# geneo4PETSc/geneo4PETSc

Measured on AMD Instinct MI355X. Metric: GenEO-PCG setup+solve sec and SpMV GB/s, 3D Laplacian 50M DoF, 1/2/4/8 GPUs, higher is better.
Workload: dtype f64

## Files before the change

### geneo4petsc_amd/csrc/amg.cpp

```cpp
#include "amg.h"

#include <algorithm>
#include <atomic>
#include <chrono>
#include <memory>
#include <cmath>
#include <cstdio>
#include <cstdlib>
#include <functional>
#include <exception>
#include <mutex>
#include <stdexcept>
#include <thread>

#include "dense.h"

namespace geneo {

static std::atomic<int> g_null_pivots{0};
int amg_null_pivots_take() { return g_null_pivots.exchange(0); }

static void parallel_rows(int n, const std::function<void(int, int)>& f) {
  int nth = std::max(1, std::min(16, (int)std::thread::hardware_concurrency()));
  if (n < 20000) nth = 1;
  if (nth == 1) {
    f(0, n);
    return;
  }
  std::vector<std::thread> th;
  for (int t = 0; t < nth; ++t)
    th.emplace_back([&, t]() { f((int)((int64_t)n * t / nth), (int)((int64_t)n * (t + 1) / nth)); });
  for (auto& x : th) x.join();
}

static HostCsr transpose_blocks(const HostCsr& a, int ncols, const std::vector<int>& rs, const std::vector<int>& cs) {
  HostCsr t;
  t.n = ncols;
  t.rowptr.assign(ncols + 1, 0);
  for (int c : a.col) t.rowptr[c + 1]++;
  for (int i = 0; i < ncols; ++i) t.rowptr[i + 1] += t.rowptr[i];
  t.col.resize(a.col.size());
  t.val.resize(a.val.size());
  const int nb = (int)rs.size() - 1;
  auto one = [&](int b) {
    std::vector<int> fill(t.rowptr.begin() + cs[b], t.rowptr.begin() + cs[b + 1]);
    for (int i = rs[b]; i < rs[b + 1]; ++i)
      for (int k = a.rowptr[i]; k < a.rowptr[i + 1]; ++k) {
        const int p = fill[a.col[k] - cs[b]]++;
        t.col[p] = i;
        t.val[p] = a.val[k];
      }
  };
  std::vector<std::thread> th;
  for (int b = 0; b < nb; ++b) th.emplace_back(one, b);
  for (auto& x : th) x.join();
  return t;
}

static HostCsr transpose(const HostCsr& a, int ncols) {
  HostCsr t;
  t.n = ncols;
  t.rowptr.assign(ncols + 1, 0);
  for (int c : a.col) t.rowptr[c + 1]++;
  for (int i = 0; i < ncols; ++i) t.rowptr[i + 1] += t.rowptr[i];
  t.col.resize(a.col.size());
  t.val.resize(a.val.size());
  std::vector<int> fill(t.rowptr.begin(), t.rowptr.end() - 1);
  for (int i = 0; i < a.n; ++i)
    for (int k = a.rowptr[i]; k < a.rowptr[i + 1]; ++k) {
      const int p = fill[a.col[k]]++;
      t.col[p] = i;
      t.val[p] = a.val[k];
    }
  return t;
}

static HostCsr spgemm(const HostCsr& a, const HostCsr& b, int ncols_b) {
  const int n = a.n;
  HostCsr c;
  c.n = n;
  c.rowptr.assign(n + 1, 0);
  int nth = std::max(1, std::min(16, (int)std::thread::hardware_concurrency()));
  if (a.col.size() < 200000) nth = 1;
  nth = std::max(1, std::min(nth, n));
  std::vector<int> cut(nth + 1, n);
  cut[0] = 0;
  for (int t = 1; t < nth; ++t) {
    const int64_t target = (int64_t)a.rowptr[n] * t / nth;
    cut[t] = (int)(std::lower_bound(a.rowptr.begin(), a.rowptr.begin() + n + 1, (int)target) - a.rowptr.begin());
    cut[t] = std::min(n, std::max(cut[t], cut[t - 1]));
  }
  auto range = [&](int t, int& r0, int& r1) {
    r0 = cut[t];
    r1 = cut[t + 1];
  };
  auto run = [&](const std::function<void(int)>& f) {
    if (nth == 1) { f(0); return; }
// ... 434 lines not shown
    } else {
      if (l == 0) throw std::runtime_error("AMG: the level-0 matrix must already be resident (fine_dev)");
      L.A = bk::csr_upload(H.A.n, H.A.rowptr.data(), H.A.col.data(), H.A.val.data());
    }
    if (l + 1 < levels.size()) {
      L.P = bk::csr_upload(H.P.n, H.P.rowptr.data(), H.P.col.data(), H.P.val.data());
      bool ok = !getenv("GENEO_AMG_UPLOAD_R");
      if (ok) {
        L.R = bk::transpose(L.P, H.R.n, &ok);
        if (ok) bk::csr_finish(L.R);
      }
      if (!ok) L.R = bk::csr_upload(H.R.n, H.R.rowptr.data(), H.R.col.data(), H.R.val.data());
    }
    L.dinv = (double*)bk::alloc(sizeof(double) * std::max(1, L.n));
    bk::h2d(L.dinv, H.dinv.data(), sizeof(double) * L.n);
    alloc_level_buffers(L, l > 0);
    L.fused = bk::csr_fusable(L.A) && (l + 1 == (int)levels.size() || bk::csr_fusable(L.P)) && !getenv("GENEO_AMG_UNFUSED");
    if (l + 1 < levels.size()) {
      make_column_scaled(L);
      make_post_matrix(L, nullptr, levels[l + 1].n);
    }
    if (l == 0) nnz0 = (double)H.nnz;
    nnzt += (double)H.nnz;
    L.suboff = H.suboff;
    lv.push_back(L);
  }
  opc = nnz0 > 0 ? nnzt / nnz0 : 1.0;
  const AmgLevelHost& C = levels.back();
  cch = bk::chunks_upload((int)C.suboff.size() - 1, C.suboff.data());
  d_inv = (double*)bk::alloc(sizeof(double) * std::max<size_t>(1, coarse_inv.size()));
  bk::h2d(d_inv, coarse_inv.data(), sizeof(double) * coarse_inv.size());
  d_invbase = (int64_t*)bk::alloc(sizeof(int64_t) * coarse_base.size());
  bk::h2d(d_invbase, coarse_base.data(), sizeof(int64_t) * coarse_base.size());
  if (prm.single) make_single();
}

void AmgDevice::make_single() {
  nlp = 0;
  for (Lvl& L : lv) {
    if (!L.fused) continue;
    const bool had = bk::csr_has_lp(L.A);
    if (bk::csr_make_lp(L.A)) ++nlp;
    L.own_lp_A = !L.own_A && !had && bk::csr_has_lp(L.A);
    if (L.Acs.n && bk::csr_make_lp(L.Acs, &L.A)) ++nlp;
    if (L.P.n && bk::csr_make_lp(L.P)) ++nlp;
    if (L.R.n && bk::csr_make_lp(L.R)) ++nlp;
    if (L.M.n && bk::csr_make_lp(L.M)) ++nlp;
  }
}

double AmgDevice::jacobi_weight(const Lvl& L) const {
  const double lmax = 1.1 * L.rho, lmin = lmax / std::max(1.5, prm.smooth_ratio);
  return 1.0 / (0.5 * (lmax + lmin));
}

void AmgDevice::make_post_matrix(Lvl& L, bk::Csr* ap, int nc) {
  const bool want = prm.smooth_degree <= 1 && L.fused && !getenv("GENEO_AMG_NO_POST_MATRIX");
  bk::Csr AP;
  bool ok = true;
  if (ap) AP = *ap;
  else if (want) AP = bk::spgemm(L.A, L.P, nc, &ok);
  if (!want || !ok || AP.n == 0) {
    if (AP.n) bk::csr_free(AP);
    return;
  }
  if (!bk::post_matrix(AP, L.P, L.dinv, jacobi_weight(L))) {
    bk::csr_free(AP);
    return;
  }
  bk::csr_finish(AP);
  if (!bk::csr_fusable(AP)) {
    bk::csr_free(AP);
    return;
  }
  L.M = AP;
}

void AmgDevice::make_column_scaled(Lvl& L) {
  if (L.fused && L.A.vec_lpr == 0 && L.A.nlong == 0 && L.A.n > 0 && !getenv("GENEO_AMG_NO_PRESCALE"))
    L.Acs = bk::csr_scaled_alias(L.A, nullptr, L.dinv, true);
}

void AmgDevice::alloc_level_buffers(Lvl& L, bool coarse) {
  const size_t blk = sizeof(double) * std::max<size_t>(1, (size_t)L.n * maxm);
  L.r = (double*)bk::alloc(blk);
  L.d = (double*)bk::alloc(blk);
  if (prm.smooth_degree > 1) L.ad = (double*)bk::alloc(blk);
  if (coarse) {
    L.b = (double*)bk::alloc(blk);
    L.x = (double*)bk::alloc(blk);
  }
}

AmgLevelHostPart amg_level_host_part(const HostCsr& Ah, const std::vector<int>& so, const AmgParams& prm, int l) {
  AmgLevelHostPart h;
  const int nsub = (int)so.size() - 1;
  const auto t_hp0 = std::chrono::high_resolution_clock::now();
  h.rho = gershgorin_rho(Ah, h.dinv, so);
  const auto t_hp1 = std::chrono::high_resolution_clock::now();
  int maxblk = 0;
  for (int s = 0; s < nsub; ++s) maxblk = std::max(maxblk, so[s + 1] - so[s]);
  h.last = (maxblk <= prm.coarse_size || l + 1 >= prm.max_levels);
  h.csub.assign(nsub + 1, 0);
  if (!h.last) {
    const int n = Ah.n;
    h.agg.assign(n, -1);
    std::vector<int> nagg(nsub, 0);
    std::vector<std::thread> th;
    for (int s = 0; s < nsub; ++s)
      th.emplace_back([&, s]() { nagg[s] = aggregate_block(Ah, so[s], so[s + 1], h.agg, amg_strength(prm, l), aggregate_threads(nsub)); });
    for (auto& x : th) x.join();
    for (int s = 0; s < nsub; ++s) h.csub[s + 1] = h.csub[s] + nagg[s];
    for (int s = 1; s < nsub; ++s) {
      const int off = h.csub[s];
      parallel_rows(so[s + 1] - so[s], [&](int a0, int a1) {
        for (int i = so[s] + a0; i < so[s] + a1; ++i) h.agg[i] += off;
      });
    }
    h.nc = h.csub[nsub];
    if (h.nc >= n) h.last = true;
  }
  if (getenv("GENEO_DEBUG") && Ah.n > 500000)
    fprintf(stderr, "[amg/host] level %d, %d rows: diagonal + bound %.3f s, aggregation %.3f s\n", l, Ah.n,
            std::chrono::duration<double>(t_hp1 - t_hp0).count(),
            std::chrono::duration<double>(std::chrono::high_resolution_clock::now() - t_hp1).count());
  return h;
}

namespace {
struct HostCsrPool {
  std::mutex mu;
  std::vector<HostCsr> parked;
  static constexpr size_t MAX_PARKED = 12;
  HostCsr take(int n, size_t nnz) {
    HostCsr out;
    {
      std::lock_guard<std::mutex> lk(mu);
      int best = -1;
      for (size_t i = 0; i < parked.size(); ++i) {
        const HostCsr& h = parked[i];
        if (h.col.size() == nnz && h.rowptr.size() == (size_t)n + 1) { best = (int)i; break; }
        if (h.col.capacity() >= nnz && h.rowptr.capacity() >= (size_t)n + 1 &&
            (best < 0 || h.col.capacity() < parked[best].col.capacity()))
          best = (int)i;
      }
      if (best >= 0) {
        out = std::move(parked[best]);
        parked.erase(parked.begin() + best);
      }
    }
    out.n = n;
    out.rowptr.resize((size_t)n + 1);
    out.col.resize(nnz);
    out.val.resize(nnz);
    return out;
  }
  void give(HostCsr&& h) {
    if (h.col.capacity() < (1u << 16)) return;
    std::lock_guard<std::mutex> lk(mu);
    if (parked.size() >= MAX_PARKED) {
      size_t k = 0;
      for (size_t i = 1; i < parked.size(); ++i)
        if (parked[i].col.capacity() < parked[k].col.capacity()) k = i;
      if (parked[k].col.capacity() >= h.col.capacity()) return;
      parked.erase(parked.begin() + k);
    }
    parked.push_back(std::move(h));
  }
};
HostCsrPool g_host_csr_pool;
}

bool AmgDevice::build_on_device(const HostCsr& A, const std::vector<int>& suboff, const AmgParams& p, int max_m,
// ... 213 lines not shown
```

### geneo4petsc_amd/csrc/backend_hip.hip

```cpp
#include <hip/hip_runtime.h>

#include <algorithm>
#include <atomic>
#include <cstdio>
#include <cstdlib>
#include <functional>
#include <stdexcept>
#include <string>
#include <chrono>
#include <condition_variable>
#include <cstring>
#include <thread>
#include <type_traits>
#include <map>
#include <mutex>
#include <unordered_map>
#include <vector>

#include "backend.h"
#include "cheb_dev.h"

#define HIPCHK(x)                                                                          \
  do {                                                                                     \
    hipError_t e_ = (x);                                                                   \
    if (e_ != hipSuccess) {                                                                \
      throw std::runtime_error(std::string("HIP error ") + hipGetErrorString(e_) + " at " + \
                               __FILE__ + ":" + std::to_string(__LINE__));                 \
    }                                                                                      \
  } while (0)

namespace bk {

static hipStream_t g_stream_main = nullptr;
static thread_local hipStream_t t_stream_side = nullptr;
static thread_local bool t_side = false;
static thread_local bool g_capturing = false;
static thread_local hipStream_t g_capture_stream = nullptr;
static std::atomic<int> g_device{-1};
static thread_local bool t_dev_bound = false;
static inline void bind_thread() {
  if (t_dev_bound) return;
  t_dev_bound = true;
  const int want = g_device.load(std::memory_order_acquire);
  if (want < 0) {
    int d = 0;
    if (hipGetDevice(&d) == hipSuccess) g_device.store(d, std::memory_order_release);
    else (void)hipGetLastError();
  } else {
    int d = -1;
    if (hipGetDevice(&d) != hipSuccess || d != want) {
      if (hipSetDevice(want) != hipSuccess) throw std::runtime_error("geneo: hipSetDevice failed on a library thread");
    }
  }
}
static inline hipStream_t stream_cur() {
  bind_thread();
  return g_capturing ? g_capture_stream : (t_side ? t_stream_side : g_stream_main);
}
#define g_stream (stream_cur())
static bool g_no_mfma = false;
static bool g_spgemm_fill_scan = getenv("GENEO_SPGEMM_SCAN_FILL") != nullptr;
static bool g_gram_flat = getenv("GENEO_GRAM_NO_FLAT") == nullptr;
static bool g_init = false;
__device__ int g_lp_no_fixed = 0;
static bool g_sell_offsets = !(getenv("GENEO_SELL_OFFSETS") && atoi(getenv("GENEO_SELL_OFFSETS")) == 0);

static void lazy_init() {
  if (g_init) return;
  g_init = true;
  const char* e = getenv("GENEO_NO_MFMA");
  g_no_mfma = (e && e[0] == '1');
  if (const char* f = getenv("GENEO_LP_FIXED")) {
    const int off = atoi(f) ? 0 : 1;
    (void)hipMemcpyToSymbol(HIP_SYMBOL(g_lp_no_fixed), &off, sizeof(int));
  }
}

const char* name() { return "hip-gfx950"; }
void set_stream(void* s) {
  if ((hipStream_t)s != g_stream_main) (void)hipStreamSynchronize(g_stream_main);
  g_stream_main = (hipStream_t)s;
  int d = 0;
  if (hipGetDevice(&d) == hipSuccess) g_device.store(d, std::memory_order_release);
  else (void)hipGetLastError();
  t_dev_bound = true;
}
void side_stream_begin(void* after, bool use_after) {
  if (t_side) return;
  bind_thread();
  if (!t_stream_side) HIPCHK(hipStreamCreateWithFlags(&t_stream_side, hipStreamNonBlocking));
  hipEvent_t ev;
  HIPCHK(hipEventCreateWithFlags(&ev, hipEventDisableTiming));
  HIPCHK(hipEventRecord(ev, use_after ? (hipStream_t)after : g_stream_main));
  HIPCHK(hipStreamWaitEvent(t_stream_side, ev, 0));
  (void)hipEventDestroy(ev);
  t_side = true;
}
void side_stream_end() {
  if (!t_side) return;
  (void)hipStreamSynchronize(t_stream_side);
  t_side = false;
  (void)hipStreamDestroy(t_stream_side);
  t_stream_side = nullptr;
}
void* get_stream() { return (void*)g_stream; }
void sync() { HIPCHK(hipStreamSynchronize(g_stream)); }

int device_count() {
  int n = 0;
  if (hipGetDeviceCount(&n) != hipSuccess) { (void)hipGetLastError(); return 0; }
  return n;
}
int set_device(int ordinal) {
  const int n = device_count();
  if (n <= 0 || ordinal < 0) return -1;
  const int d = ordinal % n;
  if (hipSetDevice(d) != hipSuccess) { (void)hipGetLastError(); return -1; }
  g_device.store(d, std::memory_order_release);
  t_dev_bound = true;
  return d;
}
int current_device() { return g_device.load(std::memory_order_acquire); }
int thread_device_check() {
  int got = -2;
  std::thread t([&]() {
    try {
      (void)stream_cur();
      int d = -1;
      if (hipGetDevice(&d) == hipSuccess) got = d;
    } catch (...) {
      got = -3;
    }
  });
  t.join();
  return got;
}
static double g_alloc_s = 0.0, g_free_s = 0.0;
static long long g_alloc_n = 0;
static std::mutex g_alloc_mu;
static std::unordered_map<void*, size_t> g_live;
struct Parked { void* p; hipStream_t stream; hipEvent_t ev; };
static std::multimap<size_t, Parked> g_cache;
static std::vector<hipEvent_t> g_ev_pool;
static size_t g_cache_bytes = 0;
static size_t g_live_bytes = 0, g_live_peak = 0, g_foot_peak = 0;
static inline void mem_account(long long delta_live) {
  g_live_bytes = (size_t)((long long)g_live_bytes + delta_live);
  g_live_peak = std::max(g_live_peak, g_live_bytes);
  g_foot_peak = std::max(g_foot_peak, g_live_bytes + g_cache_bytes);
}
static bool alloc_cache_on() {
  static const bool on = !(getenv("GENEO_ALLOC_CACHE") && !strcmp(getenv("GENEO_ALLOC_CACHE"), "0"));
  return on;
}
static size_t alloc_cache_cap() {
  static const size_t cap = (size_t)((getenv("GENEO_ALLOC_CACHE_GB") ? atof(getenv("GENEO_ALLOC_CACHE_GB")) : 96.0) * 1073741824.0);
  return cap;
}
static inline size_t alloc_round(size_t bytes) {
  const size_t g = bytes < ((size_t)1 << 20) ? 512 : ((size_t)2 << 20);
  return (bytes + g - 1) / g * g;
}
void alloc_cache_release() {
  bind_thread();
  std::lock_guard<std::mutex> lk(g_alloc_mu);
  if (g_cache.empty()) return;
  auto t0 = std::chrono::high_resolution_clock::now();
  (void)hipDeviceSynchronize();
  for (auto& kv : g_cache) {
    (void)hipFree(kv.second.p);
    if (kv.second.ev) g_ev_pool.push_back(kv.second.ev);
  }
  g_cache.clear();
  g_cache_bytes = 0;
  g_free_s += std::chrono::duration<double>(std::chrono::high_resolution_clock::now() - t0).count();
}
void* alloc(size_t bytes) {
  lazy_init();
  bind_thread();
  void* p = nullptr;
  if (bytes == 0) bytes = 8;
  const size_t sz = alloc_cache_on() ? alloc_round(bytes) : bytes;
  if (alloc_cache_on()) {
    std::lock_guard<std::mutex> lk(g_alloc_mu);
    auto it = g_cache.lower_bound(sz);
    if (it != g_cache.end() && it->first <= sz + sz / 8 + 4096) {
      p = it->second.p;
      if (it->second.ev) {
        if (it->second.stream != g_stream) (void)hipStreamWaitEvent(g_stream, it->second.ev, 0);
        g_ev_pool.push_back(it->second.ev);
      }
      g_live[p] = it->first;
      g_cache_bytes -= it->first;
      mem_account((long long)it->first);
      g_cache.erase(it);
    }
  }
  if (!p) {
    auto t0 = std::chrono::high_resolution_clock::now();
    hipError_t e = hipMalloc(&p, sz);
    if (e != hipSuccess && alloc_cache_on()) {
      (void)hipGetLastError();
      alloc_cache_release();
      e = hipMalloc(&p, sz);
    }
    HIPCHK(e);
    const double dt = std::chrono::duration<double>(std::chrono::high_resolution_clock::now() - t0).count();
    static const bool trace = getenv("GENEO_ALLOC_TRACE") != nullptr;
    if (trace && dt > 2e-4) fprintf(stderr, "[alloc] %.1f MB in %.3f ms\n", sz / 1e6, dt * 1e3);
    std::lock_guard<std::mutex> lk(g_alloc_mu);
    g_alloc_s += dt;
    ++g_alloc_n;
    g_live[p] = sz;
    mem_account((long long)sz);
  }
  HIPCHK(hipMemsetAsync(p, 0, bytes, g_stream));
  return p;
}
void dfree(void* p) {
  if (!p) return;
  bind_thread();
  {
    std::lock_guard<std::mutex> lk(g_alloc_mu);
    auto it = g_live.find(p);
    if (it != g_live.end()) {
      const size_t sz = it->second;
      g_live.erase(it);
      mem_account(-(long long)sz);
      if (alloc_cache_on() && g_cache_bytes + sz <= alloc_cache_cap()) {
        Parked pk{p, g_stream, nullptr};
        if (!g_capturing) {
          if (!g_ev_pool.empty()) { pk.ev = g_ev_pool.back(); g_ev_pool.pop_back(); }
          else if (hipEventCreateWithFlags(&pk.ev, hipEventDisableTiming) != hipSuccess) pk.ev = nullptr;
          if (pk.ev && hipEventRecord(pk.ev, g_stream) != hipSuccess) { g_ev_pool.push_back(pk.ev); pk.ev = nullptr; }
        }
        g_cache.emplace(sz, pk);
        g_cache_bytes += sz;
        return;
      }
    }
  }
  auto t0 = std::chrono::high_resolution_clock::now();
  (void)hipFree(p);
  g_free_s += std::chrono::duration<double>(std::chrono::high_resolution_clock::now() - t0).count();
}
void mem_info(double* live, double* live_peak, double* footprint_peak, double* cached, double* dev_free, double* dev_total,
              bool reset_peaks) {
  bind_thread();
  size_t f = 0, t = 0;
  if (hipMemGetInfo(&f, &t) != hipSuccess) { (void)hipGetLastError(); f = t = 0; }
  std::lock_guard<std::mutex> lk(g_alloc_mu);
  if (live) *live = (double)g_live_bytes;
  if (live_peak) *live_peak = (double)g_live_peak;
  if (footprint_peak) *footprint_peak = (double)g_foot_peak;
  if (cached) *cached = (double)g_cache_bytes;
  if (dev_free) *dev_free = (double)f;
  if (dev_total) *dev_total = (double)t;
  if (reset_peaks) {
    g_live_peak = g_live_bytes;
    g_foot_peak = g_live_bytes + g_cache_bytes;
  }
}
void alloc_stats(double* alloc_s, double* free_s, long long* n) {
  *alloc_s = g_alloc_s; *free_s = g_free_s; *n = g_alloc_n;
  g_alloc_s = g_free_s = 0.0; g_alloc_n = 0;
}
constexpr size_t STAGE_BYTES = (size_t)16 << 20;
struct StageSet {
  char* buf[2] = {nullptr, nullptr};
  hipEvent_t ev[2];
  bool ready = false, busy = false, failed = false;
};
static StageSet g_stage_sets[2];
static std::mutex g_stage_mu;
static std::condition_variable g_stage_cv;
static StageSet* stage_acquire() {
  if (getenv("GENEO_NO_PINNED_STAGING")) return nullptr;
  bind_thread();
  std::unique_lock<std::mutex> lk(g_stage_mu);
  for (;;) {
    bool any_usable = false;
    for (StageSet& st : g_stage_sets) {
      if (st.failed) continue;
      any_usable = true;
      if (st.busy) continue;
      if (!st.ready) {
        bool ok = true;
        for (int i = 0; i < 2 && ok; ++i) {
          if (hipHostMalloc((void**)&st.buf[i], STAGE_BYTES, hipHostMallocDefault) != hipSuccess) {
            (void)hipGetLastError();
            if (i == 1) (void)hipHostFree(st.buf[0]);
            st.buf[0] = st.buf[1] = nullptr;
            ok = false;
          } else if (hipEventCreateWithFlags(&st.ev[i], hipEventDisableTiming) != hipSuccess) {
            ok = false;
          }
        }
        if (!ok) { st.failed = true; continue; }
        st.ready = true;
      }
      st.busy = true;
// ... 129 lines not shown
}
void graph_destroy(void* exec) {
  if (!exec) return;
  graph_counts_drop(exec);
  (void)hipGraphExecDestroy((hipGraphExec_t)exec);
}

static inline int cdiv(int64_t a, int64_t b) { return (int)((a + b - 1) / b); }
static inline int grid1d(int64_t n, int per_block) {
  int g = cdiv(n, per_block);
  return g < 1 ? 1 : g;
}

static inline int gridv(int64_t n) { return std::min(grid1d(n, 1024), 2048); }

__device__ __forceinline__ double wave_sum(double v) {
#pragma unroll
  for (int o = 32; o > 0; o >>= 1) v += __shfl_down(v, o, 64);
  return v;
}
__device__ __forceinline__ double block_sum_256(double v, double* sm ) {
  v = wave_sum(v);
  const int w = threadIdx.x >> 6, l = threadIdx.x & 63;
  __syncthreads();
  if (l == 0) sm[w] = v;
  __syncthreads();
  return sm[0] + sm[1] + sm[2] + sm[3];
}
constexpr int SPMV_TILE = 1792;
constexpr int SPMV_ROWS = 256;
constexpr int SELL_LONG = 64;
constexpr int SELL_VEC_MAX_ROWS = 1 << 18;

__global__ void k_slice_width(const int* __restrict__ rowptr, int n, int ns, int* __restrict__ w, int long_len) {
  const int s = blockIdx.x * blockDim.x + threadIdx.x;
  if (s >= ns) return;
  int m = 0;
  const int r1 = (64 * s + 64 < n) ? 64 * s + 64 : n;
  for (int i = 64 * s; i < r1; ++i) {
    const int len = rowptr[i + 1] - rowptr[i];
    if (len <= long_len && len > m) m = len;
  }
  w[s] = m;
}
__global__ __launch_bounds__(256) void k_sell_fill(const int* __restrict__ rowptr, const int* __restrict__ col,
                                                   const double* __restrict__ val, int n, int ns,
                                                   const int64_t* __restrict__ sl_ptr, int* __restrict__ sl_col,
                                                   double* __restrict__ sl_val, int long_len) {
  const int s = blockIdx.x * 4 + (threadIdx.x >> 6);
  if (s >= ns) return;
  const int l = threadIdx.x & 63;
  const int i = 64 * s + l;
  const int64_t base = sl_ptr[s];
  const int w = (int)((sl_ptr[s + 1] - base) >> 6);
  int a = 0, len = 0;
  if (i < n) {
    a = rowptr[i];
    len = rowptr[i + 1] - a;
  }
  const bool use = (i < n) && len <= long_len;
  int padc = 0;
  if (i < n && len > 0) padc = use ? col[a + len - 1] : col[a];
  else if (n > 0 && rowptr[n] > 0) {
    const int k = (i < n) ? a : rowptr[n];
    padc = col[k > 0 ? k - 1 : 0];
  }
  for (int k = 0; k < w; ++k) {
    const int64_t e = base + (int64_t)64 * k + l;
    if (use && k < len) {
      sl_col[e] = col[a + k];
      sl_val[e] = val[a + k];
    } else {
      sl_col[e] = padc;
      sl_val[e] = 0.0;
    }
  }
}

int spmv_kind();
static bool g_force_slices = false;
static void finish_layout(Csr& a, const int* h_rowptr, const int* h_col = nullptr);

Csr csr_upload_raw(int n, const int* h_rowptr, const int* h_col, const double* h_val) {
  Csr a;
  a.n = n;
  a.nnz = h_rowptr[n];
  a.rowptr = (int*)alloc(sizeof(int) * (size_t)(n + 1));
  a.col = (int*)alloc(sizeof(int) * std::max<size_t>(1, (size_t)a.nnz));
  a.val = (double*)alloc(sizeof(double) * std::max<size_t>(1, (size_t)a.nnz));
  h2d(a.rowptr, h_rowptr, sizeof(int) * (size_t)(n + 1));
  h2d(a.col, h_col, sizeof(int) * (size_t)a.nnz);
  h2d(a.val, h_val, sizeof(double) * (size_t)a.nnz);
  return a;
}
__global__ void k_iota_ones(int* __restrict__ rp, double* __restrict__ val, int n) {
  for (int i = blockIdx.x * blockDim.x + threadIdx.x; i <= n; i += gridDim.x * blockDim.x) {
    rp[i] = i;
    if (i < n) val[i] = 1.0;
  }
}
Csr csr_tentative_prolongator(int n, const int* agg_dev) {
  Csr a;
  a.n = n;
  a.nnz = n;
  a.rowptr = (int*)alloc(sizeof(int) * (size_t)(n + 1));
  a.col = (int*)alloc(sizeof(int) * std::max<size_t>(1, (size_t)n));
  a.val = (double*)alloc(sizeof(double) * std::max<size_t>(1, (size_t)n));
  hipLaunchKernelGGL(k_iota_ones, dim3(grid1d(n + 1, 256)), dim3(256), 0, stream_cur(), a.rowptr, a.val, n);
  if (n > 0) d2d(a.col, agg_dev, sizeof(int) * (size_t)n);
  return a;
}
Csr csr_upload(int n, const int* h_rowptr, const int* h_col, const double* h_val) {
  Csr a;
  a.n = n;
  a.nnz = h_rowptr[n];
  a.rowptr = (int*)alloc(sizeof(int) * (size_t)(n + 1));
  a.col = (int*)alloc(sizeof(int) * std::max<size_t>(1, (size_t)a.nnz));
  a.val = (double*)alloc(sizeof(double) * std::max<size_t>(1, (size_t)a.nnz));
  static const bool dbg = getenv("GENEO_DEBUG") != nullptr;
  auto t0 = std::chrono::high_resolution_clock::now();
  h2d(a.rowptr, h_rowptr, sizeof(int) * (size_t)(n + 1));
  h2d(a.col, h_col, sizeof(int) * (size_t)a.nnz);
  h2d(a.val, h_val, sizeof(double) * (size_t)a.nnz);
  auto t1 = std::chrono::high_resolution_clock::now();
  finish_layout(a, h_rowptr, h_col);
  if (dbg && a.nnz > 4000000) {
    HIPCHK(hipStreamSynchronize(g_stream));
    auto t2 = std::chrono::high_resolution_clock::now();
    fprintf(stderr, "[upload] n %d nnz %lld: copies %.4f s (%.1f GB/s), layouts %.4f s\n", n, (long long)a.nnz,
            std::chrono::duration<double>(t1 - t0).count(),
            (12.0 * a.nnz + 4.0 * n) / std::chrono::duration<double>(t1 - t0).count() / 1e9,
            std::chrono::duration<double>(t2 - t1).count());
  }
  return a;
}
static std::vector<int> strip_schedule(int nslice, const std::vector<int>& frow) {
  const int WT = std::max(64, getenv("GENEO_SPMM_STRIP") ? atoi(getenv("GENEO_SPMM_STRIP")) : 3072);
  std::vector<int> order;
  order.reserve(nslice);
  int64_t covered = 0;
  std::vector<std::vector<int>> bucket;
  for (int sa = 0; sa < nslice;) {
    int sb = sa + 1;
    while (sb < nslice && frow[sb] == frow[sa]) ++sb;
    const int F = frow[sa];
    const bool swept = F >= 4 * WT && (int64_t)(sb - sa) * 64 >= (int64_t)3 * F;
    if (!swept) {
      for (int s = sa; s < sb; ++s) order.push_back(s);
    } else {
      const int nst = std::max(1, (F + WT / 2) / WT);
      const int W = (F + nst - 1) / nst;
      bucket.assign(nst, {});
      for (int s = sa; s < sb; ++s) bucket[(int)((((int64_t)(s - sa) * 64) % F) / W)].push_back(s);
      for (int b = 0; b < nst; ++b) order.insert(order.end(), bucket[b].begin(), bucket[b].end());
      covered += sb - sa;
    }
    sa = sb;
  }
  if (covered * 10 < (int64_t)nslice * 8) return {};
  if (getenv("GENEO_DEBUG_SCHED"))
    fprintf(stderr, "[sched] strip: %d slices, %lld swept, far offset of the first run %d rows, strip target %d rows\n", nslice,
            (long long)covered, frow[0], WT);
  return order;
}

static std::vector<int> blob_schedule(int n, const int* h_rowptr, const int* h_col, int nslice) {
  const int TILE = std::max(4, getenv("GENEO_SPMM_TILE") ? atoi(getenv("GENEO_SPMM_TILE")) : 512);
  const char* mode = getenv("GENEO_SPMM_SCHED");
  if (mode && !strcmp(mode, "natural")) return {};
  if (nslice < 4 * TILE) return {};
  std::vector<int> adj_ptr((size_t)nslice + 1, 0), adj;
  constexpr int CAP = 60;
  const int nth = std::max(1, std::min(8, nslice / 4096));
  std::vector<std::vector<int>> part_adj(nth);
  std::vector<int> part_far(nth, 0);
  std::vector<int> cnts((size_t)nslice, 0);
  std::vector<int> frow((size_t)nslice, 0);
  auto sample = [&](int t) {
    const int s0 = (int)((int64_t)nslice * t / nth), s1 = (int)((int64_t)nslice * (t + 1) / nth);
    std::vector<int>& out = part_adj[t];
    out.reserve((size_t)(s1 - s0) * 8);
    int far_t = 0;
    for (int s = s0; s < s1; ++s) {
      int loc[64];
      int cnt = 0;
      const int r0 = 64 * s, r1 = std::min(n, r0 + 64);
      const int probe[4] = {r0, r0 + 21, r0 + 42, r1 - 1};
      for (int t4 = 0; t4 < 4; ++t4) {
        const int r = std::min(probe[t4], r1 - 1);
        for (int k = h_rowptr[r]; k < h_rowptr[r + 1] && cnt < CAP; ++k) {
          frow[s] = std::max(frow[s], std::abs(h_col[k] - r));
          const int o = h_col[k] >> 6;
          if (o == s || o >= nslice) continue;
          bool seen = false;
          for (int i = 0; i < cnt; ++i) seen = seen || loc[i] == o;
          if (!seen) loc[cnt++] = o;
        }
      }
      for (int i = 0; i < cnt; ++i) {
        out.push_back(loc[i]);
        far_t = std::max(far_t, std::abs(loc[i] - s));
      }
      cnts[s] = cnt;
    }
    part_far[t] = far_t;
  };
  if (nth > 1) {
    std::vector<std::thread> th;
    for (int t = 1; t < nth; ++t) th.emplace_back(sample, t);
    sample(0);
    for (auto& x : th) x.join();
  } else {
    sample(0);
  }
  int far = 0;
  for (int t = 0; t < nth; ++t) far = std::max(far, part_far[t]);
  for (int s = 0; s < nslice; ++s) adj_ptr[s + 1] = adj_ptr[s] + cnts[s];
  if (!(mode && !strcmp(mode, "blob")) && far < TILE / 4) return {};
  if (!(mode && !strcmp(mode, "blob"))) {
    std::vector<int> order = strip_schedule(nslice, frow);
    if (!order.empty()) return order;
  }
  adj.reserve((size_t)adj_ptr[nslice]);
  for (int t = 0; t < nth; ++t) adj.insert(adj.end(), part_adj[t].begin(), part_adj[t].end());
  std::vector<int> order;
  order.reserve(nslice);
  std::vector<char> seen((size_t)nslice, 0);
  std::vector<int> queue;
  int next_seed = 0;
  while ((int)order.size() < nslice) {
    while (next_seed < nslice && seen[next_seed]) ++next_seed;
    if (next_seed >= nslice) break;
    queue.clear();
    queue.push_back(next_seed);
    seen[next_seed] = 1;
    size_t head = 0;
    int taken = 0;
    while (head < queue.size() && taken < TILE) {
      const int s = queue[head++];
      order.push_back(s);
      ++taken;
      for (int k = adj_ptr[s]; k < adj_ptr[s + 1]; ++k) {
        const int o = adj[k];
        if (!seen[o]) { seen[o] = 1; queue.push_back(o); }
      }
    }
    for (; head < queue.size(); ++head) seen[queue[head]] = 0;
  }
  return order;
}

static void finish_layout(Csr& a, const int* h_rowptr, const int* h_col) {
  const int n = a.n;
  static const bool dbg_l = getenv("GENEO_DEBUG") != nullptr;
  auto tl0 = std::chrono::high_resolution_clock::now();
  auto lapl = [&](const char* what) {
    if (!dbg_l || a.nnz < 4000000) return;
    HIPCHK(hipStreamSynchronize(g_stream));
    auto t = std::chrono::high_resolution_clock::now();
    fprintf(stderr, "[layout] %-22s %.4f s\n", what, std::chrono::duration<double>(t - tl0).count());
    tl0 = t;
  };
  int maxrow = 0;
  std::vector<int> longr;
  const int long_len = SELL_LONG;
  for (int i = 0; i < n; ++i) {
    const int len = h_rowptr[i + 1] - h_rowptr[i];
    maxrow = std::max(maxrow, len);
    if (len > long_len) longr.push_back(i);
  }
  a.max_row = maxrow;
  lapl("row lengths (host)");
  if (spmv_kind() == 0) {
    std::vector<int> blk;
    blk.push_back(0);
    int r = 0;
    while (r < n) {
      int r1 = r;
      int nz = 0;
      while (r1 < n && (r1 - r) < SPMV_ROWS) {
        const int len = h_rowptr[r1 + 1] - h_rowptr[r1];
        if (nz + len > SPMV_TILE) break;
        nz += len;
        ++r1;
      }
      if (r1 == r) ++r1;
      blk.push_back(r1);
      r = r1;
    }
    a.nblk = (int)blk.size() - 1;
    a.rowblk = (int*)alloc(sizeof(int) * blk.size());
    h2d(a.rowblk, blk.data(), sizeof(int) * blk.size());
  }
  {
    const int ns = (n + 63) / 64;
    int* dw = (int*)alloc(sizeof(int) * std::max(1, ns));
    if (ns > 0)
      hipLaunchKernelGGL(k_slice_width, dim3(grid1d(ns, 256)), dim3(256), 0, g_stream, a.rowptr, n, ns, dw, long_len);
    std::vector<int> w(std::max(1, ns));
    d2h(w.data(), dw, sizeof(int) * ns);
    dfree(dw);
    std::vector<int64_t> sp(ns + 1, 0);
    for (int s = 0; s < ns; ++s) sp[s + 1] = sp[s] + (int64_t)64 * w[s];
    a.nslice = ns;
    a.sl_nnz = sp[ns];
    a.sl_ptr = (int64_t*)alloc(sizeof(int64_t) * (ns + 1));
    a.sl_col = (int*)alloc(sizeof(int) * (size_t)std::max<int64_t>(1, sp[ns]));
    a.sl_val = (double*)alloc(sizeof(double) * (size_t)std::max<int64_t>(1, sp[ns]));
    h2d(a.sl_ptr, sp.data(), sizeof(int64_t) * (ns + 1));
    lapl("slice widths + scan");
    if (ns > 0)
      hipLaunchKernelGGL(k_sell_fill, dim3((ns + 3) / 4), dim3(256), 0, g_stream, a.rowptr, a.col, a.val, n, ns,
                         a.sl_ptr, a.sl_col, a.sl_val, long_len);
    lapl("slice fill");
    {
      int xp[9];
      for (int g = 0; g <= 8; ++g) xp[g] = (int)(((int64_t)ns * g) / 8);
      a.xcd_ptr = (int*)alloc(sizeof(int) * 9);
      h2d(a.xcd_ptr, xp, sizeof(int) * 9);
      if (h_col && longr.empty()) {
        const std::vector<int> order = blob_schedule(n, h_rowptr, h_col, ns);
        if ((int)order.size() == ns) {
          a.sched = (int*)alloc(sizeof(int) * (size_t)ns);
          h2d(a.sched, order.data(), sizeof(int) * (size_t)ns);
        }
      }
    }
    lapl("blob schedule");
    a.nlong = (int)longr.size();
    const double avg = n > 0 ? (double)a.nnz / n : 0.0;
    static const int vec_max_rows = getenv("GENEO_SELL_VEC_MAX_ROWS") ? atoi(getenv("GENEO_SELL_VEC_MAX_ROWS")) : SELL_VEC_MAX_ROWS;
    if (!g_force_slices && n < vec_max_rows && (a.nlong > 0 || avg >= 20.0)) a.vec_lpr = avg <= 24.0 ? 16 : (avg <= 48.0 ? 32 : 64);
    a.long_rows = (int*)alloc(sizeof(int) * std::max<size_t>(1, longr.size()));
    h2d(a.long_rows, longr.data(), sizeof(int) * longr.size());
  }
// ... 307 lines not shown
    const unsigned long long prev = __shfl_up(ck, 1, 64);
    const bool head = (ck != ~0ull) && (lane == 0 || (prev >> 6) != (ck >> 6));
    double acc = 0.0 + v;
    for (int d = 1; d < 64; ++d) {
      const unsigned long long nk = __shfl_down(ck, d, 64);
      const double nv = __shfl_down(v, d, 64);
      const bool more = head && lane + d < 64 && (nk >> 6) == (ck >> 6);
      if (more) acc += nv;
      if (!__ballot(more)) break;
    }
    const unsigned long long heads = __ballot(head);
    if (head) {
      const int pos = __builtin_popcountll(heads & ((1ull << lane) - 1ull));
      ccol[base + pos] = (int)(ck >> 6);
      cval[base + pos] = acc;
    }
    return;
  }
  spg_collect(arp, acol, brp, bcol, row, lane, keys[w], ja[w], pre[w], total, overflow);
  const int* kw = keys[w];
  double* hv = hval[w];
  for (int s = lane; s < SPG_HS; s += 64) hv[s] = 0.0;
  if (lane == 0) cntl[w] = 0;
  for (int t = lane; t < SPG_MAXD; t += 64) list[w][t] = 0x7fffffff;
  __builtin_amdgcn_fence(__ATOMIC_ACQ_REL, "wavefront");
  __builtin_amdgcn_wave_barrier();
  const int a0 = arp[row], na = arp[row + 1] - a0;
  if (total >= 0) {
    constexpr int NB = 4;
    for (int p0 = 0; p0 < total; p0 += 64 * NB) {
      int kk[NB], slot[NB];
      double vv[NB];
#pragma unroll
      for (int t = 0; t < NB; ++t) {
        const int p = p0 + 64 * t + lane;
        kk[t] = (p < total) ? spg_find(pre[w], na, p) : 0x7fffffff;
      }
#pragma unroll
      for (int t = 0; t < NB; ++t) {
        slot[t] = 0;
        vv[t] = 0.0;
        if (kk[t] != 0x7fffffff) {
          const int l = brp[ja[w][kk[t]]] + (p0 + 64 * t + lane - pre[w][kk[t]]);
          slot[t] = bcol[l];
          vv[t] = aval[a0 + kk[t]] * bval[l];
        }
      }
#pragma unroll
      for (int t = 0; t < NB; ++t)
        if (kk[t] != 0x7fffffff) slot[t] = spg_lookup(kw, slot[t]);
#pragma unroll
      for (int t = 0; t < NB; ++t) {
        if (p0 + 64 * t >= total) break;
        int kc = __builtin_amdgcn_readfirstlane(kk[t]);
        while (true) {
          if (kk[t] == kc) hv[slot[t]] += vv[t];
          __builtin_amdgcn_fence(__ATOMIC_ACQ_REL, "wavefront");
          const unsigned long long later = __ballot(kk[t] != 0x7fffffff && kk[t] > kc);
          if (!later) break;
          kc = __shfl(kk[t], __builtin_ctzll(later), 64);
        }
      }
    }
  } else {
    for (int k = a0; k < a0 + na; ++k) {
      const int j = acol[k];
      const double av = aval[k];
      for (int l = brp[j] + lane; l < brp[j + 1]; l += 64) hv[spg_lookup(kw, bcol[l])] += av * bval[l];
      __builtin_amdgcn_fence(__ATOMIC_ACQ_REL, "wavefront");
    }
  }
  __builtin_amdgcn_fence(__ATOMIC_ACQ_REL, "wavefront");
  __builtin_amdgcn_wave_barrier();
  for (int s = lane; s < SPG_HS; s += 64) {
    const int key = kw[s];
    if (key != -1) {
      const int t = atomicAdd(&cntl[w], 1);
      list[w][t] = key;
      lval[w][t] = hv[s];
    }
  }
  __builtin_amdgcn_fence(__ATOMIC_ACQ_REL, "wavefront");
  __builtin_amdgcn_wave_barrier();
  int N = 64;
  while (N < cnt) N <<= 1;
  wave_bitonic_sort(list[w], lval[w], N, lane);
  for (int t = lane; t < cnt; t += 64) {
    ccol[base + t] = list[w][t];
    cval[base + t] = lval[w][t];
  }
}
template <int G, bool FILL>
__global__ __launch_bounds__(256) void k_spgemm_small(int n, const int* __restrict__ arp, const int* __restrict__ acol,
                                                      const double* __restrict__ aval, const int* __restrict__ brp,
                                                      const int* __restrict__ bcol, const double* __restrict__ bval,
                                                      int* __restrict__ cnt, const int* __restrict__ crp,
                                                      int* __restrict__ ccol, double* __restrict__ cval,
                                                      unsigned char* __restrict__ defer, int* __restrict__ flags) {
  constexpr int RPW = 64 / G;
  const int w = threadIdx.x >> 6, lane = threadIdx.x & 63;
  const int gl = lane % G, gbase = lane - gl;
  const int row = (blockIdx.x * 4 + w) * RPW + lane / G;
  const bool live = row < n;
  const int a0 = live ? arp[row] : 0;
  const int na = live ? arp[row + 1] - a0 : 0;
  int b0 = 0, len = 0;
  double av = 0.0;
  if (gl < na && na <= G) {
    const int j = acol[a0 + gl];
    b0 = brp[j];
    len = brp[j + 1] - b0;
    if (FILL) av = aval[a0 + gl];
  }
  int incl = len;
#pragma unroll
  for (int o = 1; o < G; o <<= 1) {
    const int t = __shfl_up(incl, o, G);
    if (gl >= o) incl += t;
  }
  const int total = __shfl(incl, G - 1, G);
  const bool fits = na <= G && total <= G;
  if (!FILL && live && gl == 0) {
    defer[row] = fits ? 0 : 1;
    if (!fits) atomicAdd(&flags[1], 1);
  }
  int k = 0;
#pragma unroll
  for (int q = 0; q < G; ++q) k += (__shfl(incl, q, G) <= gl) ? 1 : 0;
  const bool has = fits && gl < total;
  const int ks = has ? k : 0;
  const int kb0 = __shfl(b0, ks, G);
  const int kexcl = __shfl(incl - len, ks, G);
  double kav = 0.0;
  if (FILL) kav = __shfl(av, ks, G);
  unsigned long long ck = ~0ull;
  double v = 0.0;
  if (has) {
    const int l = kb0 + (gl - kexcl);
    ck = ((unsigned long long)(unsigned)bcol[l] << 6) | (unsigned)gl;
    if (FILL) v = kav * bval[l];
  }
#pragma unroll
  for (int k2 = 2; k2 <= G; k2 <<= 1)
#pragma unroll
    for (int j = k2 >> 1; j > 0; j >>= 1) {
      const unsigned long long ock = __shfl_xor(ck, j, 64);
      double ov = 0.0;
      if (FILL) ov = __shfl_xor(v, j, 64);
      const bool take_min = (((gl & j) == 0) == ((gl & k2) == 0));
      const bool swap = take_min ? (ock < ck) : (ock > ck);
      if (swap) { ck = ock; if (FILL) v = ov; }
    }
  const unsigned long long prev = __shfl_up(ck, 1, G);
  const bool head = (ck != ~0ull) && (gl == 0 || (prev >> 6) != (ck >> 6));
  const unsigned long long gmask = (G == 64) ? ~0ull : (((1ull << G) - 1ull) << gbase);
  const unsigned long long heads = __ballot(head) & gmask;
  if (!FILL) {
    if (live && fits && gl == 0) cnt[row] = __builtin_popcountll(heads);
    return;
  }
  double acc = 0.0 + v;
  for (int d = 1; d < G; ++d) {
    const unsigned long long nk = __shfl_down(ck, d, G);
    const double nv = __shfl_down(v, d, G);
    const bool more = head && gl + d < G && (nk >> 6) == (ck >> 6);
    if (more) acc += nv;
// ... 36 lines not shown
  }
  if (t == 255) totals[blockIdx.x] = part[255];
}
__global__ __launch_bounds__(256) void k_scan_blocks64(int64_t* __restrict__ x, int64_t n, int64_t* __restrict__ totals) {
  __shared__ int64_t part[256];
  const int64_t b0 = (int64_t)blockIdx.x * SCAN_B;
  const int t = threadIdx.x;
  int64_t v[4], run = 0;
#pragma unroll
  for (int u = 0; u < 4; ++u) {
    const int64_t i = b0 + 4 * t + u;
    run += (i < n) ? x[i] : 0;
    v[u] = run;
  }
  part[t] = run;
  __syncthreads();
  for (int o = 1; o < 256; o <<= 1) {
    const int64_t add = (t >= o) ? part[t - o] : 0;
    __syncthreads();
    part[t] += add;
    __syncthreads();
  }
  const int64_t before = (t > 0) ? part[t - 1] : 0;
#pragma unroll
  for (int u = 0; u < 4; ++u) {
    const int64_t i = b0 + 4 * t + u;
    if (i < n) x[i] = before + v[u];
  }
  if (t == 255) totals[blockIdx.x] = part[255];
}
__global__ void k_scan_add(int* __restrict__ x, int64_t n, const int64_t* __restrict__ totals_incl) {
  for (int64_t i = (int64_t)blockIdx.x * blockDim.x + threadIdx.x + SCAN_B; i < n; i += (int64_t)gridDim.x * blockDim.x)
    x[i] += (int)totals_incl[i / SCAN_B - 1];
}
__global__ void k_scan_add64(int64_t* __restrict__ x, int64_t n, const int64_t* __restrict__ totals_incl) {
  for (int64_t i = (int64_t)blockIdx.x * blockDim.x + threadIdx.x + SCAN_B; i < n; i += (int64_t)gridDim.x * blockDim.x)
    x[i] += totals_incl[i / SCAN_B - 1];
}
static void device_inclusive_scan64(int64_t* x, int64_t n) {
  if (n <= 0) return;
  const int64_t nb = (n + SCAN_B - 1) / SCAN_B;
  int64_t* tot = (int64_t*)alloc(sizeof(int64_t) * (size_t)nb);
  hipLaunchKernelGGL(k_scan_blocks64, dim3((unsigned)nb), dim3(256), 0, g_stream, x, n, tot);
  if (nb > 1) {
    t_sp_report.scan_depth = 2;
    device_inclusive_scan64(tot, nb);
    hipLaunchKernelGGL(k_scan_add64, dim3((unsigned)std::min<int64_t>(nb, 4096)), dim3(256), 0, g_stream, x, n, tot);
  }
  dfree(tot);
}
static void host_exclusive_scan(int* dcnt_to_ptr, int n, int64_t* total) {
  if (n <= 0) { *total = 0; return; }
  static const bool on_host = getenv("GENEO_SCAN_HOST") != nullptr;
  if (on_host || (int64_t)n < 4 * SCAN_B) {
    std::vector<int> h((size_t)n + 1, 0);
    d2h(h.data() + 1, dcnt_to_ptr + 1, sizeof(int) * (size_t)n);
    int64_t run = 0;
    for (int i = 1; i <= n; ++i) {
      run += h[i];
      h[i] = (int)run;
    }
    h[0] = 0;
    h2d(dcnt_to_ptr, h.data(), sizeof(int) * ((size_t)n + 1));
    *total = run;
    return;
  }
  int* x = dcnt_to_ptr + 1;
  t_sp_report.scan_depth = 1;
  const int64_t nb = ((int64_t)n + SCAN_B - 1) / SCAN_B;
  int64_t* tot = (int64_t*)alloc(sizeof(int64_t) * (size_t)nb);
  hipLaunchKernelGGL(k_scan_blocks, dim3((unsigned)nb), dim3(256), 0, g_stream, x, (int64_t)n, tot);
  device_inclusive_scan64(tot, nb);
  hipLaunchKernelGGL(k_scan_add, dim3((unsigned)std::min<int64_t>(nb, 4096)), dim3(256), 0, g_stream, x, (int64_t)n, tot);
  HIPCHK(hipMemsetAsync(dcnt_to_ptr, 0, sizeof(int), g_stream));
  int64_t run = 0;
  d2h(&run, tot + (nb - 1), sizeof(int64_t));
  dfree(tot);
  if (run > 0x7fffffffLL) throw std::runtime_error("sparse product: more than 2^31 entries");
  *total = run;
}
static bool g_spgemm_small_host = true;
Csr spgemm(const Csr& a, const Csr& b, int ncols_b, bool* ok) {
  (void)ncols_b;
  Csr c;
  *ok = true;
  t_sp_report = SparseProductReport();
  c.n = a.n;
  if (a.n == 0) return c;
  int* dflag = (int*)alloc(2 * sizeof(int));
  c.rowptr = (int*)alloc(sizeof(int) * ((size_t)a.n + 1));
  int G = 0;
  if (g_spgemm_small_host && !g_spgemm_fill_scan && a.n >= 256 && b.n > 0) {
    const double na = (double)a.nnz / a.n, est = na * ((double)b.nnz / b.n);
    if (na <= 7.5 && est <= 7.5) G = 8;
    else if (na <= 15.0 && est <= 14.0) G = 16;
    else if (na <= 30.0 && est <= 26.0) G = 32;
    else if (na <= 60.0 && est <= 52.0) G = 64;
  }
  t_sp_report.group = G;
  unsigned char* defer = nullptr;
#define SPG_SMALL(GG, FILL)                                                                                                  \
  hipLaunchKernelGGL((k_spgemm_small<GG, FILL>), dim3((unsigned)((a.n + 256 / GG - 1) / (256 / GG))), dim3(256), 0, g_stream, \
                     a.n, a.rowptr, a.col, a.val, b.rowptr, b.col, b.val, c.rowptr + 1, c.rowptr, c.col, c.val, defer, dflag)
#define SPG_SMALL_G(FILL)                                      \
  do {                                                         \
    if (G == 8) SPG_SMALL(8, FILL);                            \
    else if (G == 16) SPG_SMALL(16, FILL);                     \
    else if (G == 32) SPG_SMALL(32, FILL);                     \
    else SPG_SMALL(64, FILL);                                  \
  } while (0)
  int hflag[2] = {0, 0};
  if (G) {
    defer = (unsigned char*)alloc((size_t)a.n);
    SPG_SMALL_G(false);
    d2h(hflag, dflag, 2 * sizeof(int));
    t_sp_report.deferred = hflag[1];
  }
  const bool general = !G || hflag[1] > 0;
  if (general) {
    hipLaunchKernelGGL(k_spgemm_count, dim3((a.n + 3) / 4), dim3(256), 0, g_stream, a.n, a.rowptr, a.col, b.rowptr, b.col,
                       c.rowptr + 1, dflag, defer);
    d2h(hflag, dflag, sizeof(int));
  }
  if (hflag[0]) {
    dfree(dflag);
    dfree(defer);
    dfree(c.rowptr);
    *ok = false;
    return Csr();
  }
  int64_t total = 0;
  host_exclusive_scan(c.rowptr, a.n, &total);
  c.nnz = total;
  c.col = (int*)alloc(sizeof(int) * std::max<size_t>(1, (size_t)total));
  c.val = (double*)alloc(sizeof(double) * std::max<size_t>(1, (size_t)total));
  if (G) SPG_SMALL_G(true);
  if (general) {
    if (g_spgemm_fill_scan)
      hipLaunchKernelGGL(k_spgemm_fill_scan, dim3((a.n + 3) / 4), dim3(256), 0, g_stream, a.n, a.rowptr, a.col, a.val, b.rowptr,
                         b.col, b.val, c.rowptr, c.col, c.val, dflag);
    else
      hipLaunchKernelGGL(k_spgemm_fill, dim3((a.n + 3) / 4), dim3(256), 0, g_stream, a.n, a.rowptr, a.col, a.val, b.rowptr,
                         b.col, b.val, c.rowptr, c.col, c.val, dflag, defer);
    d2h(hflag, dflag, sizeof(int));
  }
#undef SPG_SMALL_G
#undef SPG_SMALL
  dfree(dflag);
  dfree(defer);
  if (hflag[0]) {
    dfree(c.rowptr); dfree(c.col); dfree(c.val);
    *ok = false;
    return Csr();
  }
  return c;
}

constexpr int TR_MAXROW = 1024;
__global__ void k_col_count(const int* __restrict__ col, int64_t nnz, int* __restrict__ cnt) {
  for (int64_t e = (int64_t)blockIdx.x * blockDim.x + threadIdx.x; e < nnz; e += (int64_t)gridDim.x * blockDim.x)
    atomicAdd(&cnt[col[e]], 1);
}
__global__ void k_tr_scatter(int n, const int* __restrict__ rp, const int* __restrict__ col, const double* __restrict__ val,
                             const int* __restrict__ trp, int* __restrict__ cursor, int* __restrict__ tcol,
                             double* __restrict__ tval) {
  for (int i = blockIdx.x * blockDim.x + threadIdx.x; i < n; i += gridDim.x * blockDim.x)
    for (int k = rp[i]; k < rp[i + 1]; ++k) {
      const int c = col[k];
      const int p = trp[c] + atomicAdd(&cursor[c], 1);
      tcol[p] = i;
      tval[p] = val[k];
    }
}
__global__ __launch_bounds__(256) void k_sort_rows(int n, const int* __restrict__ rp, int* __restrict__ col,
                                                   double* __restrict__ val, int* __restrict__ overflow) {
  __shared__ int key[4][TR_MAXROW];
  __shared__ double v[4][TR_MAXROW];
  const int w = threadIdx.x >> 6, lane = threadIdx.x & 63;
  const int row = blockIdx.x * 4 + w;
  if (row >= n) return;
  const int base = rp[row], cnt = rp[row + 1] - base;
  if (cnt <= 1) return;
  if (cnt > TR_MAXROW) {
    if (lane == 0) *overflow = 1;
    return;
  }
  int N = 64;
  while (N < cnt) N <<= 1;
  for (int t = lane; t < N; t += 64) {
    key[w][t] = (t < cnt) ? col[base + t] : 0x7fffffff;
    v[w][t] = (t < cnt) ? val[base + t] : 0.0;
  }
  __builtin_amdgcn_wave_barrier();
  wave_bitonic_sort(key[w], v[w], N, lane);
  for (int t = lane; t < cnt; t += 64) {
    col[base + t] = key[w][t];
    val[base + t] = v[w][t];
  }
}
Csr transpose(const Csr& a, int ncols, bool* ok) {
  Csr t;
  *ok = true;
  t_sp_report = SparseProductReport();
  t.n = ncols;
  t.nnz = a.nnz;
  t.rowptr = (int*)alloc(sizeof(int) * ((size_t)ncols + 1));
  t.col = (int*)alloc(sizeof(int) * std::max<size_t>(1, (size_t)a.nnz));
  t.val = (double*)alloc(sizeof(double) * std::max<size_t>(1, (size_t)a.nnz));
  if (a.nnz > 0)
    hipLaunchKernelGGL(k_col_count, dim3(gridv(a.nnz)), dim3(256), 0, g_stream, a.col, (int64_t)a.nnz, t.rowptr + 1);
  int64_t total = 0;
  host_exclusive_scan(t.rowptr, ncols, &total);
  int* cursor = (int*)alloc(sizeof(int) * std::max<size_t>(1, (size_t)ncols));
  int* dflag = (int*)alloc(sizeof(int));
  if (a.n > 0)
    hipLaunchKernelGGL(k_tr_scatter, dim3(gridv(a.n)), dim3(256), 0, g_stream, a.n, a.rowptr, a.col, a.val, t.rowptr,
                       cursor, t.col, t.val);
  if (ncols > 0)
    hipLaunchKernelGGL(k_sort_rows, dim3((ncols + 3) / 4), dim3(256), 0, g_stream, ncols, t.rowptr, t.col, t.val, dflag);
  int hflag = 0;
  d2h(&hflag, dflag, sizeof(int));
  dfree(dflag);
  dfree(cursor);
  if (hflag) {
    dfree(t.rowptr); dfree(t.col); dfree(t.val);
    *ok = false;
    return Csr();
  }
  return t;
}
__global__ void k_smooth_p(int n, const int* __restrict__ rp, const int* __restrict__ col, double* __restrict__ val,
                           const int* __restrict__ agg, const double* __restrict__ dinv, double w) {
  for (int i = blockIdx.x * blockDim.x + threadIdx.x; i < n; i += gridDim.x * blockDim.x) {
    const double f = -w * dinv[i];
    const int mine = agg[i];
    for (int k = rp[i]; k < rp[i + 1]; ++k) val[k] = f * val[k] + (col[k] == mine ? 1.0 : 0.0);
  }
}
void smooth_prolongator(Csr& ap0, const int* agg_dev, const double* dinv_dev, double w) {
  if (ap0.n == 0) return;
  hipLaunchKernelGGL(k_smooth_p, dim3(gridv(ap0.n)), dim3(256), 0, g_stream, ap0.n, ap0.rowptr, ap0.col, ap0.val, agg_dev,
                     dinv_dev, w);
}

__global__ void k_post_matrix(int n, const int* __restrict__ arp, const int* __restrict__ acol, double* __restrict__ aval,
                              const int* __restrict__ prp, const int* __restrict__ pcol, const double* __restrict__ pval,
                              const double* __restrict__ dinv, double w, int* __restrict__ miss) {
  for (int i = blockIdx.x * blockDim.x + threadIdx.x; i < n; i += gridDim.x * blockDim.x) {
    const int p0 = prp[i], p1 = prp[i + 1];
    const double f = w * dinv[i];
    int found = 0;
    for (int k = arp[i]; k < arp[i + 1]; ++k) {
      const int c = acol[k];
      double v = -f * aval[k];
      for (int q = p0; q < p1; ++q)
        if (pcol[q] == c) { v += pval[q]; ++found; break; }
      aval[k] = v;
    }
    if (found != p1 - p0) atomicExch(miss, 1);
  }
}
bool post_matrix(Csr& ap, const Csr& p, const double* dinv, double w) {
  if (ap.n == 0) return true;
  int* dmiss = (int*)alloc(sizeof(int));
  hipLaunchKernelGGL(k_post_matrix, dim3(gridv(ap.n)), dim3(256), 0, g_stream, ap.n, ap.rowptr, ap.col, ap.val, p.rowptr,
                     p.col, p.val, dinv, w, dmiss);
  int miss = 0;
  d2h(&miss, dmiss, sizeof(int));
  dfree(dmiss);
  return miss == 0;
}

void csr_free_lp(Csr& a) {
  dfree(a.lp_val);
  if (!a.alias) { dfree(a.lp_col); dfree(a.lp_base); dfree(a.off_mask); dfree(a.off_rec); }
  a.lp_val = nullptr; a.lp_col = nullptr; a.lp_base = nullptr;
  a.off_mask = nullptr; a.off_rec = nullptr; a.off_coded = 0; a.off_nnz = 0;
}
void csr_free(Csr& a) {
  csr_free_lp(a);
  if (a.alias) {
    dfree(a.val); dfree(a.sl_val);
    a = Csr();
    return;
  }
  dfree(a.rowptr); dfree(a.col); dfree(a.val); dfree(a.rowblk);
  dfree(a.sl_ptr); dfree(a.sl_col); dfree(a.sl_val); dfree(a.long_rows);
  dfree(a.sched); dfree(a.xcd_ptr);
  a = Csr();
}

__global__ void k_scale_csr(int n, const int* __restrict__ rowptr, const int* __restrict__ col, const double* __restrict__ val,
                            const double* __restrict__ rs, const double* __restrict__ cs, double* __restrict__ out) {
  const int r = blockIdx.x * blockDim.x + threadIdx.x;
  if (r >= n) return;
  const double a = rs ? rs[r] : 1.0;
  for (int k = rowptr[r]; k < rowptr[r + 1]; ++k) out[k] = a * val[k] * (cs ? cs[col[k]] : 1.0);
}
__global__ __launch_bounds__(256) void k_scale_sell(int n, int ns, const int64_t* __restrict__ sl_ptr,
                                                    const int* __restrict__ sl_col, const double* __restrict__ sl_val,
                                                    const double* __restrict__ rs, const double* __restrict__ cs,
                                                    double* __restrict__ out) {
  const int s = blockIdx.x * 4 + (threadIdx.x >> 6);
  if (s >= ns) return;
  const int l = threadIdx.x & 63;
  const int r = 64 * s + l;
  const double a = (rs && r < n) ? rs[r] : 1.0;
  for (int64_t e = sl_ptr[s] + l; e < sl_ptr[s + 1]; e += 64) out[e] = a * sl_val[e] * (cs ? cs[sl_col[e]] : 1.0);
}
Csr csr_scaled_alias(const Csr& a, const double* row_scale, const double* col_scale, bool col_is_dinv) {
  Csr b = a;
  b.alias = true;
  b.lp_val = nullptr; b.lp_col = nullptr; b.lp_base = nullptr;
  b.off_mask = nullptr; b.off_rec = nullptr; b.off_coded = 0; b.off_nnz = 0;
  b.col_scaled = col_is_dinv;
  b.val = (double*)alloc(sizeof(double) * std::max<size_t>(1, (size_t)a.nnz));
  b.sl_val = (double*)alloc(sizeof(double) * (size_t)std::max<int64_t>(1, a.sl_nnz));
  if (a.n > 0)
    hipLaunchKernelGGL(k_scale_csr, dim3(grid1d(a.n, 256)), dim3(256), 0, g_stream, a.n, a.rowptr, a.col, a.val, row_scale,
                       col_scale, b.val);
  if (a.nslice > 0)
    hipLaunchKernelGGL(k_scale_sell, dim3((a.nslice + 3) / 4), dim3(256), 0, g_stream, a.n, a.nslice, a.sl_ptr, a.sl_col,
                       a.sl_val, row_scale, col_scale, b.sl_val);
  return b;
}

__device__ __forceinline__ int xcd_remap(int b, int nblk) {
  const int per = (nblk + 7) >> 3;
  const int t = (b & 7) * per + (b >> 3);
  return t;
}

__global__ __launch_bounds__(256) void k_spmv_lds(const int* __restrict__ rowblk, int nblk,
                                                  const int* __restrict__ rowptr,
                                                  const int* __restrict__ col,
                                                  const double* __restrict__ val,
                                                  const double* __restrict__ x, double* __restrict__ y) {
  __shared__ double prod[SPMV_TILE];
  const int t = xcd_remap(blockIdx.x, nblk);
  if (t >= nblk) return;
  const int r0 = rowblk[t], r1 = rowblk[t + 1];
  const int nz0 = rowptr[r0], nz1 = rowptr[r1];
  const int cnt = nz1 - nz0;
  const int tid = threadIdx.x;
  if (cnt > SPMV_TILE) {
    double s = 0.0;
    for (int k = nz0 + tid; k < nz1; k += 256) s += val[k] * x[col[k]];
    prod[tid] = s;
    __syncthreads();
    for (int w = 128; w > 0; w >>= 1) {
      if (tid < w) prod[tid] += prod[tid + w];
      __syncthreads();
    }
    if (tid == 0) y[r0] = prod[0];
    return;
  }
  for (int k = tid; k < cnt; k += 256) prod[k] = val[nz0 + k] * x[col[nz0 + k]];
  __syncthreads();
  const int r = r0 + tid;
  if (r < r1) {
    const int a = rowptr[r] - nz0, b = rowptr[r + 1] - nz0;
    double s = 0.0;
    for (int k = a; k < b; ++k) s += prod[k];
    y[r] = s;
  }
}

__device__ __forceinline__ int4 lp_base_of(const int* __restrict__ base, int s) {
  return base ? reinterpret_cast<const int4*>(base)[s] : int4{0, 0, 0x7fffffff, 0};
}
template <typename COLT, bool NT>
struct ColsStored {
  const COLT* __restrict__ col;
  int4 cb;
  __device__ __forceinline__ int at(int u, int64_t e0) const {
    return (u < cb.z ? cb.x : cb.y) + (int)(NT ? __builtin_nontemporal_load(col + e0 + 64 * u) : col[e0 + 64 * u]);
  }
  template <int KW>
  __device__ __forceinline__ void finish(int (&)[KW]) const {}
};
constexpr int OFF_NONE = (int)0x80000000;
struct ColsOffset {
  int4 o0, o1;
  unsigned char m8;
  int ov;
  int r, pad;
  __device__ __forceinline__ int at(int, int64_t) const { return 0; }
  template <int KW>
  __device__ __forceinline__ void finish(int (&c)[KW]) const {
    constexpr unsigned full = (1u << KW) - 1u;
    const unsigned m = m8;
    const int off[8] = {o0.x, o0.y, o0.z, o0.w, o1.x, o1.y, o1.z, o1.w};
    if (__ballot(m != full) == 0) {
#pragma unroll
      for (int u = 0; u < KW; ++u) c[u] = r + off[u];
    } else {
      unsigned mm = m;
#pragma unroll
      for (int u = 0; u < KW; ++u) {
// ... 452 lines not shown
  const int s = blockIdx.x * 4 + (threadIdx.x >> 6);
  if (s >= ns) return;
  const int l = threadIdx.x & 63;
  const int r = 64 * s + l;
  const int64_t a = sl_ptr[s];
  const int wd = (int)((sl_ptr[s + 1] - a) >> 6);
  int len = r < n ? rowptr[r + 1] - rowptr[r] : 0;
  bool ok = wd >= 1 && wd <= 8 && __ballot(len > wd) == 0;
  if (!ok) len = 0;
  int d[8];
  int hi = -1;
#pragma unroll
  for (int k = 0; k < 8; ++k) {
    d[k] = 0;
    if (k < len) {
      const int c = sl_col[a + 64 * (int64_t)k + l];
      d[k] = c - r;
      hi = c > hi ? c : hi;
    }
  }
  hi = lp_wave_max(hi);
  int offs[8];
  int nd = 0, last = OFF_NONE;
#pragma unroll
  for (int it = 0; it < 9; ++it) {
    int mine = 0x7fffffff;
#pragma unroll
    for (int k = 0; k < 8; ++k)
      if (k < len && d[k] > last && d[k] < mine) mine = d[k];
    const int m = lp_wave_min(mine);
    const bool found = m != 0x7fffffff;
    if (it < 8) {
      offs[it < 8 ? it : 0] = found ? m : 0;
      if (found) nd = it + 1;
    } else if (found) {
      ok = false;
    }
    if (found) last = m;
  }
  unsigned msk = 0;
  int prev = -1;
  bool bad = false;
#pragma unroll
  for (int k = 0; k < 8; ++k) {
    if (k < len) {
      int slot = -1;
#pragma unroll
      for (int j = 0; j < 8; ++j)
        if (j < nd && offs[j] == d[k]) slot = j;
      if (slot <= prev) bad = true;
      else msk |= 1u << slot;
      prev = slot;
    }
  }
  const int pad = r < n ? r : n - 1;
  unsigned mm = bad ? 0u : msk;
#pragma unroll
  for (int k = 0; k < 8; ++k) {
    if (k < wd && ok) {
      int c = pad;
      if (mm) {
        const int slot = __ffs(mm) - 1;
        int o = 0;
#pragma unroll
        for (int j = 0; j < 8; ++j)
          if (j == slot) o = offs[j];
        c = r + o;
        mm &= mm - 1u;
      }
      if (k < len ? c != sl_col[a + 64 * (int64_t)k + l] : (c < 0 || c > hi)) bad = true;
    }
  }
  ok = ok && __ballot(bad) == 0;
  mask[r] = ok ? (unsigned char)msk : (unsigned char)0;
#pragma unroll
  for (int j = 0; j < 8; ++j)
    if (l == j) rec[8 * (int64_t)s + j] = ok ? offs[j] : OFF_NONE;
  if (ok && l == 0) {
    atomicAdd(cnt, 1ull);
    atomicAdd(cnt + 1, (unsigned long long)wd * 64ull);
  }
}
bool csr_make_lp(Csr& a, const Csr* index_owner) {
  if (spmv_kind() != 1 || a.nslice == 0 || !a.sl_ptr || a.vec_lpr > 0 || a.nlong > 0 || a.lp_val) return a.lp_val != nullptr;
  if (index_owner) {
    if (!index_owner->lp_val || index_owner->sl_col != a.sl_col) return false;
    a.lp_col = index_owner->lp_col;
    a.lp_base = index_owner->lp_base;
    a.off_mask = index_owner->off_mask;
    a.off_rec = index_owner->off_rec;
    a.off_coded = index_owner->off_coded;
    a.off_nnz = index_owner->off_nnz;
  } else {
    const char* lim_env = getenv("GENEO_LP_SPAN_MAX");
    int limit = lim_env ? atoi(lim_env) : 65535;
    if (limit < 1 || limit > 65535) limit = 65535;
    a.lp_base = (int*)alloc(sizeof(int4) * (size_t)a.nslice);
    unsigned long long* dstat = (unsigned long long*)alloc(3 * sizeof(unsigned long long));
    HIPCHK(hipMemsetAsync(dstat, 0, 3 * sizeof(unsigned long long), g_stream));
    int* dfail = (int*)dstat;
    unsigned long long* dcnt = dstat + 1;
    hipLaunchKernelGGL(k_lp_base, dim3((a.nslice + 3) / 4), dim3(256), 0, g_stream, a.nslice, a.sl_ptr, a.sl_col,
                       (int4*)a.lp_base, dfail, limit, dfail + 1);
    const double avg_w = (double)a.sl_nnz / (64.0 * (double)a.nslice);
    const bool off_try = a.rowptr && (a.max_row <= 8 || avg_w - 8.0 <= 0.1 * ((double)a.max_row - 8.0));
    if (off_try) {
      a.off_mask = (unsigned char*)alloc((size_t)64 * (size_t)a.nslice);
      a.off_rec = (int*)alloc(sizeof(int) * 8 * (size_t)a.nslice);
      hipLaunchKernelGGL(k_off_code, dim3((a.nslice + 3) / 4), dim3(256), 0, g_stream, a.nslice, a.n, a.rowptr, a.sl_ptr,
                         a.sl_col, a.off_mask, a.off_rec, dcnt);
    }
    unsigned long long hstat[3] = {0, 0, 0};
    d2h(hstat, dstat, sizeof(hstat));
    dfree(dstat);
    int hfail[2];
    memcpy(hfail, &hstat[0], sizeof(hfail));
    const unsigned long long* hcnt = hstat + 1;
    if (hfail[0]) {
      dfree(a.lp_base);
      a.lp_base = nullptr;
    } else {
      a.lp_col = (unsigned short*)alloc(sizeof(unsigned short) * (size_t)std::max<int64_t>(1, a.sl_nnz));
      a.off_coded = (int)hcnt[0];
      a.off_nnz = (int64_t)hcnt[1];
    }
    const bool off_use = a.lp_col && a.off_coded > 0 && 10 * (int64_t)a.off_coded >= 9 * (int64_t)a.nslice;
    if (!off_use) {
      dfree(a.off_mask);
      dfree(a.off_rec);
      a.off_mask = nullptr;
      a.off_rec = nullptr;
    }
    if (getenv("GENEO_DEBUG"))
      fprintf(stderr, "[offsets] %d-row matrix, %d slices, %d coded%s\n", a.n, a.nslice, a.off_coded,
              !off_try ? " (too wide: not tried)" : off_use ? "" : (a.off_coded ? " (under 90 %: stored columns kept)" : ""));
    if (getenv("GENEO_DEBUG") && (hfail[0] || hfail[1]))
      fprintf(stderr, "[lp] %d-row matrix, %d slices: %s (span limit %d)\n", a.n, a.nslice,
              hfail[0] ? "32-bit columns kept (a slice needs more than two bases)"
                       : (std::to_string(hfail[1]) + " slices with two column bases").c_str(), limit);
  }
  a.lp_val = (float*)alloc(sizeof(float) * (size_t)std::max<int64_t>(1, a.sl_nnz));
  hipLaunchKernelGGL(k_lp_fill, dim3((a.nslice + 3) / 4), dim3(256), 0, g_stream, a.nslice, a.sl_ptr, a.sl_col, a.sl_val,
                     (const int4*)a.lp_base, (index_owner || !a.lp_col) ? (unsigned short*)nullptr : a.lp_col, a.lp_val);
  return true;
}
template <int EPI, int WPS, typename COLT, bool NT, bool OFFS = false>
__global__ __launch_bounds__(256) void k_spmv_sell_lp(const int64_t* __restrict__ sl_ptr, int nslice, int n,
                                                      const COLT* __restrict__ col, const float* __restrict__ val,
                                                      const int* __restrict__ base, const double* __restrict__ x,
                                                      double* __restrict__ y, const double* __restrict__ b,
                                                      double* __restrict__ z, const double* __restrict__ dinv, double w,
                                                      const double* __restrict__ cs,
                                                      const unsigned char* __restrict__ omask = nullptr,
                                                      const int* __restrict__ orec = nullptr) {
  spmv_sell_slice<float, COLT, EPI, WPS, NT, OFFS, SliceLp>(sl_ptr, nslice, n, col, val, base, x, y, b, z, dinv, w, cs, omask,
                                                            orec);
}
struct LpArgs {
  const double* x;
  double* y;
  const double* b;
  double* z;
  const double* dinv;
  double w;
  const double* cs;
};
// ... 630 lines not shown
          }
          d2 res;
          res.x = mk.x * (acc1[u].x - lm.x * acc2[u].x);
          res.y = mk.y * (acc1[u].y - lm.y * acc2[u].y);
          __builtin_nontemporal_store(res, reinterpret_cast<d2*>(Y1 + r * ldy + 2 * q));
        } else {
          __builtin_nontemporal_store(acc1[u], reinterpret_cast<d2*>(Y1 + r * ldy + 2 * q));
          __builtin_nontemporal_store(acc2[u], reinterpret_cast<d2*>(Y2 + r * ldy + 2 * q));
        }
      }
    }
  }
}
bool spmm_dual_available(const Csr& a, int m) {
  if (spmv_kind() != 1 || a.vec_lpr > 0 || a.nlong > 0 || !a.sl_ptr || !a.xcd_ptr || sell_wide_mm(a)) return false;
  return m == 16 || m == 32 || m == 64;
}
void spmm_dual(const Csr& a, const double* v1, const double* v2, const double* X, int ldx, double* Y1, double* Y2, int ldy,
               int m) {
  if (a.n == 0) return;
  if (!spmm_dual_available(a, m) || (ldx & 1) || (ldy & 1) || !aligned16(X) || !aligned16(Y1) || !aligned16(Y2))
    throw std::runtime_error("spmm_dual: operands not on the sliced path");
  ProfScope prof(PROF_SPMM, a.fine && m >= 16, (double)a.nnz * 20.0 + (double)a.n * 4.0 + 24.0 * m * (double)a.n,
                 4.0 * (double)a.nnz * m);
  int wpx = g_spmm_wpx < 0 ? 64 : (g_spmm_wpx == 0 ? 64 : g_spmm_wpx);
  const int need = (a.nslice + 31) / 32;
  if (wpx > need) wpx = need < 1 ? 1 : need;
#define DUAL(L)                                                                                                   \
  hipLaunchKernelGGL((k_spmm_sell_dual<L, 2, 0>), dim3(8 * wpx), dim3(256), 0, g_stream, a.sl_ptr, a.sl_col, v1, v2, a.n,  \
                     a.sched, a.xcd_ptr, X, ldx, Y1, Y2, ldy, (const int*)nullptr, 0, (const double*)nullptr,            \
                     (const double*)nullptr)
  if (m == 16) DUAL(8);
  else if (m == 32) DUAL(16);
  else DUAL(32);
#undef DUAL
}
void spmm_dual_residual(const Csr& a, const double* v1, const double* v2, const double* X, int ldx, double* R, int ldr,
                        int m, const Chunks& c, const double* lam, const double* mask) {
  if (a.n == 0) return;
  if (!spmm_dual_available(a, m) || (ldx & 1) || (ldr & 1) || !aligned16(X) || !aligned16(R) || !aligned16(lam) || !aligned16(mask))
    throw std::runtime_error("spmm_dual_residual: operands not on the sliced path");
  if (c.n != a.n) throw std::runtime_error("spmm_dual_residual: the subdomain list does not cover the matrix rows");
  ProfScope prof(PROF_SPMM, a.fine && m >= 16, (double)a.nnz * 20.0 + (double)a.n * 4.0 + 16.0 * m * (double)a.n,
                 4.0 * (double)a.nnz * m);
  int wpx = g_spmm_wpx < 0 ? 64 : (g_spmm_wpx == 0 ? 64 : g_spmm_wpx);
  const int need = (a.nslice + 31) / 32;
  if (wpx > need) wpx = need < 1 ? 1 : need;
#define DUALR(L)                                                                                                  \
  hipLaunchKernelGGL((k_spmm_sell_dual<L, 2, 1>), dim3(8 * wpx), dim3(256), 0, g_stream, a.sl_ptr, a.sl_col, v1, v2, a.n,  \
                     a.sched, a.xcd_ptr, X, ldx, R, (double*)nullptr, ldr, c.suboff, c.nsub, lam, mask)
  if (m == 16) DUALR(8);
  else if (m == 32) DUALR(16);
  else DUALR(32);
#undef DUALR
}
__global__ __launch_bounds__(256) void k_sell_values_on(int n, int ns, const int64_t* __restrict__ sl_ptr,
                                                        const int* __restrict__ sl_col, const int* __restrict__ arp,
                                                        const int* __restrict__ brp, const int* __restrict__ bcol,
                                                        const double* __restrict__ bval, double* __restrict__ out,
                                                        int* __restrict__ missing) {
  const int s = blockIdx.x * 4 + (threadIdx.x >> 6);
  if (s >= ns) return;
  const int l = threadIdx.x & 63;
  const int r = 64 * s + l;
  const int64_t base = sl_ptr[s];
  const int wd = (int)((sl_ptr[s + 1] - base) >> 6);
  const int la = r < n ? arp[r + 1] - arp[r] : 0;
  const int b0 = r < n ? brp[r] : 0, b1 = r < n ? brp[r + 1] : 0;
  int found = 0;
  for (int k = 0; k < wd; ++k) {
    const int64_t e = base + (int64_t)64 * k + l;
    double v = 0.0;
    if (k < la) {
      const int c = sl_col[e];
      for (int t = b0; t < b1; ++t)
        if (bcol[t] == c) { v = bval[t]; ++found; break; }
    }
    out[e] = v;
  }
  if (found != b1 - b0) atomicAdd(missing, 1);
}
double* sell_values_on(const Csr& a, const Csr& b) {
  if (spmv_kind() != 1 || a.nlong > 0 || a.vec_lpr > 0 || !a.sl_ptr || a.n != b.n || a.nslice == 0) return nullptr;
  double* out = (double*)alloc(sizeof(double) * (size_t)std::max<int64_t>(1, a.sl_nnz));
  int* dmiss = (int*)alloc(sizeof(int));
  hipLaunchKernelGGL(k_sell_values_on, dim3((a.nslice + 3) / 4), dim3(256), 0, g_stream, a.n, a.nslice, a.sl_ptr, a.sl_col,
                     a.rowptr, b.rowptr, b.col, b.val, out, dmiss);
  int h = 0;
  d2h(&h, dmiss, sizeof(int));
  dfree(dmiss);
  if (h) {
    dfree(out);
    return nullptr;
  }
  return out;
}

static void spmm_ld(const Csr& a, const double* X, int ldx, double* Y, int ldy, int m, const double* pre,
                    const double* post) {
  if (a.n == 0 || m == 0) return;
  ProfScope prof(PROF_SPMM, a.fine && m >= 16, (double)a.nnz * 12.0 + (double)a.n * 4.0 + 16.0 * m * (double)a.n,
                 2.0 * (double)a.nnz * m);
  if (spmm_sell_launch<EPI_NONE>(a, X, ldx, Y, ldy, m, pre, post, nullptr, 0, nullptr, 0, nullptr, 0.0)) return;
  if (m <= 16) {
    int g = std::min(grid1d(a.n, 16), 8192);
    hipLaunchKernelGGL(k_spmm<16>, dim3(g), dim3(256), 0, g_stream, a.n, a.rowptr, a.col, a.val, X, ldx, Y,
                       ldy, m, pre, post);
  } else if (m <= 32) {
    int g = std::min(grid1d(a.n, 8), 8192);
    hipLaunchKernelGGL(k_spmm<32>, dim3(g), dim3(256), 0, g_stream, a.n, a.rowptr, a.col, a.val, X, ldx, Y,
                       ldy, m, pre, post);
  } else {
    int g = std::min(grid1d(a.n, 4), 8192);
    hipLaunchKernelGGL(k_spmm<64>, dim3(g), dim3(256), 0, g_stream, a.n, a.rowptr, a.col, a.val, X, ldx, Y,
                       ldy, m, pre, post);
  }
}
void spmm_strided(const Csr& a, const double* X, int ldx, double* Y, int ldy, int m, const double* pre,
                  const double* post) {
  spmm_ld(a, X, ldx, Y, ldy, m, pre, post);
}

bool csr_fusable(const Csr& a) { return spmv_kind() == 1 && (a.vec_lpr > 0 || a.nlong == 0); }

template <int EPI>
static void spmm_fused_t(const Csr& a, const double* X, int ldx, double* Y, int ldy, int m, const double* B, int ldb,
                         double* Z, int ldz, const double* dinv, double w) {
  if (m == 1 && ldx <= 1 && ldy == 1 && ldb <= 1 && ldz <= 1 && csr_fusable(a)) {
    if (a.vec_lpr > 0) {
      spmv_vec_launch<EPI>(a, X, Y, B, Z, dinv, w);
      return;
    }
    if (sell_wide(a)) {
      spmv_wide_launch<EPI>(a, X, Y, B, Z, dinv, w);
      return;
    }
    const int nwb = (a.nslice + 3) / 4;
    const int perw = (nwb + 7) / 8;
    hipLaunchKernelGGL((k_spmv_sell_epi<false, EPI>), dim3(perw * 8), dim3(256), 0, g_stream, a.sl_ptr, a.nslice,
                       a.n, a.sl_col, a.sl_val, X, Y, B, Z, dinv, w, a.col_scaled ? (const double*)nullptr : dinv);
    return;
  }
  const double* Xin = (EPI == EPI_PRE) ? B : X;
  const int ldin = (EPI == EPI_PRE) ? ldb : ldx;
  const double* pre = (EPI == EPI_PRE && !a.col_scaled) ? dinv : nullptr;
  ProfScope prof(PROF_SPMM, a.fine && m >= 16,
                 (double)a.nnz * 12.0 + (double)a.n * 4.0 + (16.0 + ((EPI == EPI_JAC || EPI == EPI_POST) ? 16.0 : 8.0)) * m * (double)a.n,
                 2.0 * (double)a.nnz * m);
  if (spmm_sell_launch<EPI>(a, Xin, ldin, Y, ldy, m, pre, nullptr, B, ldb, Z, ldz, dinv, w)) return;
  if (m <= 16) {
    int g = std::min(grid1d(a.n, 16), 8192);
    hipLaunchKernelGGL((k_spmm<16, EPI>), dim3(g), dim3(256), 0, g_stream, a.n, a.rowptr, a.col, a.val, Xin, ldin, Y,
                       ldy, m, pre, nullptr, B, ldb, Z, ldz, dinv, w);
  } else if (m <= 32) {
    int g = std::min(grid1d(a.n, 8), 8192);
    hipLaunchKernelGGL((k_spmm<32, EPI>), dim3(g), dim3(256), 0, g_stream, a.n, a.rowptr, a.col, a.val, Xin, ldin, Y,
                       ldy, m, pre, nullptr, B, ldb, Z, ldz, dinv, w);
  } else {
    int g = std::min(grid1d(a.n, 4), 8192);
    hipLaunchKernelGGL((k_spmm<64, EPI>), dim3(g), dim3(256), 0, g_stream, a.n, a.rowptr, a.col, a.val, Xin, ldin, Y,
                       ldy, m, pre, nullptr, B, ldb, Z, ldz, dinv, w);
  }
}
void spmm_fused(const Csr& a, int epi, const double* X, int ldx, double* Y, int ldy, int m, const double* B, int ldb,
                double* Z, int ldz, const double* dinv, double w) {
  if (a.n == 0 || m == 0) return;
// ... 1502 lines not shown
}
void dense_sym_apply(const Chunks& c, const double* inv, const int64_t* base, const double* B, int ldb, double* X,
                     int ldx, int m) {
  if (c.nchunk == 0) return;
  hipLaunchKernelGGL(k_dense_sym_apply, dim3(c.nchunk), dim3(256), 0, g_stream, c.start, c.len, c.sub, c.suboff, inv,
                     base, B, ldb, X, ldx, m);
}

template <int PB>
__global__ __launch_bounds__(1024) void k_chol_solve(const double* __restrict__ L, const double* __restrict__ LT, int n,
                                                     double* __restrict__ y) {
  extern __shared__ double xs[];
  const int t = threadIdx.x;
  double yv = (t < n) ? y[t] : 0.0;
  const double dg = (t < n) ? L[(int64_t)t * n + t] : 1.0;
  for (int k0 = 0; k0 < n; k0 += PB) {
    double c[PB];
#pragma unroll
    for (int p = 0; p < PB; ++p) {
      const int k = k0 + p;
      c[p] = (k < n && t > k && t < n) ? LT[(int64_t)k * n + t] : 0.0;
    }
#pragma unroll
    for (int p = 0; p < PB; ++p) {
      const int k = k0 + p;
      if (k < n) {
        if (t == k) { yv = yv / dg; xs[k] = yv; }
        __syncthreads();
        if (t > k) yv -= c[p] * xs[k];
      }
    }
  }
  for (int k0 = 0; k0 < n; k0 += PB) {
    double c[PB];
#pragma unroll
    for (int p = 0; p < PB; ++p) {
      const int k = n - 1 - (k0 + p);
      c[p] = (k >= 0 && t < k) ? L[(int64_t)k * n + t] : 0.0;
    }
#pragma unroll
    for (int p = 0; p < PB; ++p) {
      const int k = n - 1 - (k0 + p);
      if (k >= 0) {
        if (t == k) { yv = yv / dg; xs[k] = yv; }
        __syncthreads();
        if (t < k) yv -= c[p] * xs[k];
      }
    }
  }
  if (t < n) y[t] = yv;
}
bool chol_solve(const double* L, const double* LT, int n, double* y) {
  if (n <= 0) return true;
  if (n > 1024) return false;
  const int threads = ((n + 63) / 64) * 64;
  hipLaunchKernelGGL((k_chol_solve<16>), dim3(1), dim3(threads), sizeof(double) * n, g_stream, L, LT, n, y);
  return true;
}

__global__ void k_mfma_selftest(double* out) {
  const int l = threadIdx.x;
  const int i = l & 15, k = l >> 4;
  const double a = (i == k) ? 1.0 : 0.0;
  const double b = 100.0 * k + (l & 15);
  d4 acc = (d4){0.0, 0.0, 0.0, 0.0};
  acc = __builtin_amdgcn_mfma_f64_16x16x4f64(a, b, acc, 0, 0, 0);
  for (int v = 0; v < 4; ++v) {
    const int row = (l >> 4) + 4 * v, colj = l & 15;
    out[row * 16 + colj] = acc[v];
  }
}
void set_mfma(bool enable) { lazy_init(); g_no_mfma = !enable; }
bool set_variant(const char* name, int value) {
  const std::string k(name ? name : "");
  if (k == "spgemm_fill_scan") { g_spgemm_fill_scan = value != 0; return true; }
  if (k == "gram_flat") { g_gram_flat = value != 0; return true; }
  if (k == "lp_fixed") {
    lazy_init();
    const int off = value ? 0 : 1;
    HIPCHK(hipMemcpyToSymbol(HIP_SYMBOL(g_lp_no_fixed), &off, sizeof(int)));
    return true;
  }
  if (k == "sell_offsets") { g_sell_offsets = value != 0; return true; }
  if (k == "spgemm_small_rows") {
    lazy_init();
    const int off = value ? 0 : 1;
    HIPCHK(hipMemcpyToSymbol(HIP_SYMBOL(g_spgemm_no_small), &off, sizeof(int)));
    g_spgemm_small_host = value != 0;
    return true;
  }
  return false;
}
int selftest_mfma_f64() {
  double* d = (double*)alloc(sizeof(double) * 256);
  hipLaunchKernelGGL(k_mfma_selftest, dim3(1), dim3(64), 0, g_stream, d);
  double h[256];
  d2h(h, d, sizeof(h));
  dfree(d);
  for (int i = 0; i < 16; ++i)
    for (int j = 0; j < 16; ++j) {
      const double want = (i < 4) ? 100.0 * i + j : 0.0;
      if (h[i * 16 + j] != want) return 1 + i * 16 + j;
    }
  return 0;
}

void* event_create() {
  hipEvent_t e;
  HIPCHK(hipEventCreate(&e));
  return (void*)e;
}
void event_record(void* ev) { HIPCHK(hipEventRecord((hipEvent_t)ev, g_stream)); }
static hipStream_t g_copy_stream = nullptr;
void d2h_after(void* host, const void* dev, size_t bytes, void* event) {
  if (!bytes) return;
  if (!g_copy_stream) HIPCHK(hipStreamCreateWithFlags(&g_copy_stream, hipStreamNonBlocking));
  HIPCHK(hipStreamWaitEvent(g_copy_stream, (hipEvent_t)event, 0));
  HIPCHK(hipMemcpyAsync(host, dev, bytes, hipMemcpyDeviceToHost, g_copy_stream));
  HIPCHK(hipStreamSynchronize(g_copy_stream));
}
float event_elapsed_ms(void* a, void* b) {
  HIPCHK(hipEventSynchronize((hipEvent_t)b));
  float ms = 0.f;
  HIPCHK(hipEventElapsedTime(&ms, (hipEvent_t)a, (hipEvent_t)b));
  return ms;
}
void event_destroy(void* ev) {
  if (ev) (void)hipEventDestroy((hipEvent_t)ev);
}

}
```

### geneo4petsc_amd/csrc/core.cpp

```cpp
#include "core.h"

#include <algorithm>
#include <atomic>
#include <chrono>
#include <cfloat>
#include <cmath>
#include <cstdio>
#include <cstdlib>
#include <cstring>
#include <condition_variable>
#include <exception>
#include <mutex>
#include <functional>
#include <future>
#include <map>
#include <numeric>
#include <fstream>
#include <iomanip>
#include <sstream>
#include <stdexcept>
#include <thread>

#include "amg.h"
#include "block_dev.h"
#include "cheb_dev.h"
#include "coarse_dev.h"
#include "dense.h"
#include "gmres_col.h"

namespace bk {
__attribute__((weak)) bool coarse_factor(const double*, int, int, double*, double*, int*) { return false; }
__attribute__((weak)) bool coarse_solve(const double*, const double*, int, int, double*) { return false; }
__attribute__((weak)) bool coarse_solve_block(const double*, const double*, int, int, double*, int) { return false; }
__attribute__((weak)) SparseProductReport sparse_product_report() { return SparseProductReport(); }
}

namespace geneo {
static std::atomic<int> g_cheb_fused{1}, g_block_fused{1};
void set_cheb_fused(int on) { g_cheb_fused = on ? 1 : 0; }
int cheb_fused() { return g_cheb_fused.load(); }
void set_block_fused(int on) { g_block_fused = on ? 1 : 0; }
int block_fused() { return g_block_fused.load(); }
static int step_fused(int w) { return w == 1 ? g_cheb_fused.load() : g_block_fused.load(); }

static int slab_entries(int n, int w) {
  if ((int64_t)n * w > 0x7fffffffll) throw std::runtime_error("GenEO: a slab of right-hand sides exceeds 2^31 entries");
  return n * w;
}

void StepWork::alloc(int n_, int ns_, int w_) {
  release();
  if (n_ <= 0 || ns_ <= 0 || w_ <= 0) return;
  t = (double*)bk::alloc(sizeof(double) * (size_t)n_ * w_);
  ab = (double*)bk::alloc(sizeof(double) * 2 * (size_t)ns_ * w_);
  idx = (int*)bk::alloc(sizeof(int) * 2 * (size_t)ns_ * w_);
  std::vector<int> h(2 * (size_t)ns_ * w_);
  for (int s = 0; s < ns_; ++s)
    for (int j = 0; j < w_; ++j) {
      h[(size_t)s * w_ + j] = 2 * s;
      h[(size_t)ns_ * w_ + (size_t)s * w_ + j] = 2 * s + 1;
    }
  bk::h2d(idx, h.data(), sizeof(int) * h.size());
  n = n_;
  ns = ns_;
  w = w_;
}
void StepWork::release() {
  bk::dfree(t);
  bk::dfree(ab);
  bk::dfree(idx);
  t = ab = nullptr;
  idx = nullptr;
  n = ns = w = 0;
}

bool cheb_dir_composed(const bk::Chunks& c, const double* coef_k, int flags, const double* Z, double* D, double* X,
                       const double* dscale, double* Out, int w, const StepWork& wk) {
  const int n = c.n, ns = c.nsub;
  if (n <= 0 || ns <= 0) return true;
  if (wk.n < n || wk.ns != ns || wk.w != w) throw std::runtime_error("cheb_dir_composed: scratch of another size");
  const int nw = slab_entries(n, w);
  bk::gather(wk.ab, coef_k, wk.idx, 2 * ns * w);
  if (flags & 1) {
    bk::copy(D, Z, nw);
    bk::block_colscale(c, D, w, w, wk.ab);
    bk::copy(X, D, nw);
  } else {
    bk::copy(wk.t, Z, nw);
    bk::block_colscale(c, wk.t, w, w, wk.ab);
    bk::block_colscale(c, D, w, w, wk.ab + (size_t)ns * w);
    bk::axpy(D, 1.0, wk.t, nw);
    bk::axpy(X, 1.0, D, nw);
  }
  if (flags & 2) {
    if (dscale) bk::block_rowscale(Out, w, X, w, dscale, 1.0, 0.0, n, w);
    else bk::copy(Out, X, nw);
  }
  return true;
}

bool cheb_dir_composed_once(const bk::Chunks& c, const double* coef_k, int flags, const double* Z, double* D, double* X,
                            const double* dscale, double* Out, int w) {
  struct Own {
    StepWork w;
    ~Own() { w.release(); }
  } own;
  own.w.alloc(c.n, c.nsub, w);
  const bool ok = cheb_dir_composed(c, coef_k, flags, Z, D, X, dscale, Out, w, own.w);
  bk::sync();
  return ok;
}

bool block_import_composed(const double* Xcm, int ld, int n, int m, double* Yrm, int w) {
  if (n <= 0) return true;
  bk::zero(Yrm, sizeof(double) * (size_t)n * w);
  for (int j = 0; j < m; ++j) bk::block_axpby(Yrm + j, w, 1.0, Xcm + (size_t)j * ld, 1, 0.0, n, 1);
  return true;
// ... 495 lines not shown
    std::atomic<int> bad{0};
    parallel_ranges((int64_t)nL, [&](int64_t i0, int64_t i1) {
      int s = (int)(std::upper_bound(suboff.begin(), suboff.end(), (int)i0) - suboff.begin()) - 1;
      for (int64_t i = i0; i < i1;) {
        while (s + 1 < ns && i >= suboff[s + 1]) ++s;
        const std::vector<int>& l2g = subs[s].l2g;
        const int64_t e1 = std::min<int64_t>(i1, suboff[s + 1]);
        for (; i < e1; ++i) {
          const int g = l2g[i - suboff[s]];
          int e = -1;
          if (g < 0 || g >= N) { bad = 1; return; }
          if (ident) e = g;
          else {
            auto it = std::lower_bound(owned.begin(), owned.end(), g);
            if (it != owned.end() && *it == g) e = (int)(it - owned.begin());
            else {
              auto h = std::lower_bound(hmap.begin(), hmap.end(), std::make_pair(g, -1));
              if (h == hmap.end() || h->first != g) { bad = 2; return; }
              e = nown + h->second;
            }
          }
          l2e[i] = e;
        }
      }
    });
    if (bad == 1) return fail("GenEO preconditioner: global index out of range");
    if (bad == 2) return fail("GenEO preconditioner: DOF neither owned nor in the halo plan");
  }
  d_l2e = (int*)bk::alloc(sizeof(int) * std::max(1, nL));
  bk::h2d(d_l2e, l2e.data(), sizeof(int) * nL);
  bool rt_done = false;
  if (nL > 0 && !getenv("GENEO_RT_HOST")) {
    bk::Csr Rm = bk::csr_tentative_prolongator(nL, d_l2e);
    bool ok = false;
    bk::Csr Rt = bk::transpose(Rm, nE, &ok);
    bk::csr_free(Rm);
    if (ok) {
      d_rt_ptr = Rt.rowptr;
      d_rt_idx = Rt.col;
      bk::dfree(Rt.val);
      rt_done = true;
    }
  }
  if (!rt_done) {
    std::vector<int> rt_ptr(nE + 1, 0), rt_idx(nL);
    for (int j = 0; j < nL; ++j) rt_ptr[l2e[j] + 1]++;
    for (int e = 0; e < nE; ++e) rt_ptr[e + 1] += rt_ptr[e];
    {
      std::vector<int> fill(rt_ptr.begin(), rt_ptr.end() - 1);
      for (int j = 0; j < nL; ++j) rt_idx[fill[l2e[j]]++] = j;
    }
    d_rt_ptr = (int*)bk::alloc(sizeof(int) * (nE + 1));
    d_rt_idx = (int*)bk::alloc(sizeof(int) * std::max(1, nL));
    bk::h2d(d_rt_ptr, rt_ptr.data(), sizeof(int) * (nE + 1));
    bk::h2d(d_rt_idx, rt_idx.data(), sizeof(int) * nL);
  }
  const int nsend = (int)send_idx.size();
  if (size > 1) {
    if ((int)recv_counts.size() != size || (int)send_counts.size() != size) return fail("GenEO: bad halo plan");
    if (std::accumulate(recv_counts.begin(), recv_counts.end(), 0) != nH) return fail("GenEO: bad halo recv counts");
    if (std::accumulate(send_counts.begin(), send_counts.end(), 0) != nsend) return fail("GenEO: bad halo send counts");
    if (!cb_exchange || !cb_allreduce || !comm_send || !comm_recv || !comm_red) return fail("GenEO: communicator not set");
    d_send_idx = (int*)bk::alloc(sizeof(int) * std::max(1, nsend));
    bk::h2d(d_send_idx, send_idx.data(), sizeof(int) * nsend);
    std::vector<int> rv_ptr(nown + 1, 0), rv_idx(nsend);
    for (int k = 0; k < nsend; ++k) {
      if (send_idx[k] < 0 || send_idx[k] >= nown) return fail("GenEO: bad halo send index");
      rv_ptr[send_idx[k] + 1]++;
    }
    for (int e = 0; e < nown; ++e) rv_ptr[e + 1] += rv_ptr[e];
    std::vector<int> fill(rv_ptr.begin(), rv_ptr.end() - 1);
    for (int k = 0; k < nsend; ++k) rv_idx[fill[send_idx[k]]++] = k;
    d_rv_ptr = (int*)bk::alloc(sizeof(int) * (nown + 1));
    d_rv_idx = (int*)bk::alloc(sizeof(int) * std::max(1, nsend));
    bk::h2d(d_rv_ptr, rv_ptr.data(), sizeof(int) * (nown + 1));
    bk::h2d(d_rv_idx, rv_idx.data(), sizeof(int) * nsend);
    n_rv = nsend;
  }
  ch = bk::chunks_upload(ns, suboff.data());
  std::vector<int> gids(std::max(1, ns));
  for (int s = 0; s < ns; ++s) gids[s] = subs[s].gid;
  d_subgid = (int*)bk::alloc(sizeof(int) * std::max(1, ns));
  bk::h2d(d_subgid, gids.data(), sizeof(int) * ns);
  auto dv = [](size_t n) { return (double*)bk::alloc(sizeof(double) * std::max<size_t>(1, n)); };
  d_xe = dv(nE); d_ye = dv(nE); d_xL = dv(nL); d_wL = dv(nL);
  d_cg_r = dv(nL); d_cg_z = dv(nL); d_cg_p = dv(nL); d_cg_q = dv(nL); d_cg_sc = dv((size_t)8 * std::max(1, ns));
  d_t1 = dv(nown); d_t2 = dv(nown); d_t3 = dv(nown); d_x0 = dv(nown); d_scal = dv(16);
  vec.w = 1;
  vec.coarse = true;
  vec.wl = d_wL; vec.xl = d_xL; vec.r1 = d_cg_r; vec.z = d_cg_z; vec.d = d_cg_p;
  vec.t1 = d_t1; vec.t2 = d_t2; vec.t3 = d_t3;
  vec.xe = d_xe; vec.ye = d_ye;
  vec.work = &cheb_work;
  vec.chain = &cheb_chain;
  return 0;
}

int PC::ensure_dirichlet() {
  bool missing = false;
  for (auto& s : subs)
    if (s.a_dir.empty()) missing = true;
  if (!missing) return 0;
  if (size > 1)
    return fail("GenEO preconditioner without dirichlet matrix (pass pcADirLoc when subdomains span several ranks)");
  size_t tot = 0;
  for (auto& s : subs) tot += s.a_neu.val.size();
  struct Ent { int64_t key; double v; };
  std::vector<Ent> coo;
  coo.reserve(tot);
  for (auto& s : subs)
    for (int i = 0; i < s.a_neu.n; ++i)
      for (int k = s.a_neu.rowptr[i]; k < s.a_neu.rowptr[i + 1]; ++k)
        coo.push_back({(int64_t)s.l2g[i] * N + s.l2g[s.a_neu.col[k]], s.a_neu.val[k]});
  std::stable_sort(coo.begin(), coo.end(), [](const Ent& a, const Ent& b) { return a.key < b.key; });
  std::vector<int64_t> keys;
  std::vector<double> vals;
  keys.reserve(coo.size());
  vals.reserve(coo.size());
  for (size_t i = 0; i < coo.size();) {
    size_t j = i;
    double v = 0.0;
    while (j < coo.size() && coo[j].key == coo[i].key) v += coo[j++].v;
    keys.push_back(coo[i].key);
    vals.push_back(v);
    i = j;
  }
  std::vector<int64_t> rowstart(N + 1, 0);
  for (int64_t k : keys) rowstart[k / N + 1]++;
  for (int i = 0; i < N; ++i) rowstart[i + 1] += rowstart[i];
  std::vector<int> g2l(N, -1);
  for (auto& s : subs) {
    if (!s.a_dir.empty()) continue;
    const int n = (int)s.l2g.size();
    for (int i = 0; i < n; ++i) g2l[s.l2g[i]] = i;
    s.a_dir.n = n;
    s.a_dir.rowptr.assign(n + 1, 0);
    s.a_dir.col.clear();
    s.a_dir.val.clear();
    for (int i = 0; i < n; ++i) {
      const int g = s.l2g[i];
      for (int64_t k = rowstart[g]; k < rowstart[g + 1]; ++k) {
        const int gc = (int)(keys[k] % N);
        if (g2l[gc] >= 0) {
          s.a_dir.col.push_back(g2l[gc]);
          s.a_dir.val.push_back(vals[k]);
        }
      }
      s.a_dir.rowptr[i + 1] = (int)s.a_dir.col.size();
    }
    for (int i = 0; i < n; ++i) g2l[s.l2g[i]] = -1;
  }
  return 0;
}

void PC::make_robin(Sub& s, HostCsr& out) const {
  out = s.a_dir;
  if (std::fabs(opt.optim) <= DBL_EPSILON) return;
  const int n = (int)s.l2g.size();
  std::vector<std::map<int, double>> rows(n);
  for (int i = 0; i < n; ++i)
    for (int k = s.a_dir.rowptr[i]; k < s.a_dir.rowptr[i + 1]; ++k) rows[i][s.a_dir.col[k]] += s.a_dir.val[k];
  for (int i = 0; i < n; ++i) {
    if (s.mult[i] <= 1) continue;
    for (int k = s.a_neu.rowptr[i]; k < s.a_neu.rowptr[i + 1]; ++k) {
      const int c = s.a_neu.col[k];
      if (s.mult[c] > 1) rows[i][c] += opt.optim * s.a_neu.val[k];
// ... 680 lines not shown
    done = true;
    for (int s = 0; s < ns; ++s) {
      if (sc[(size_t)s * 8 + 6] != 0.0) done = false;
      else if (dbg_dls1 && conv_at[s] < 0) conv_at[s] = it;
    }
  };
  static const bool adaptive = !getenv("GENEO_DLS1_FIXED_CHUNKS");
  if (use_amg && adaptive && cg_long_len >= 8 && check % 2 == 0) {
    const int first = cg_long_len;
    run(first);
    const int64_t single_rows = getenv("GENEO_DLS1_SINGLE_STEP_ROWS") ? atoll(getenv("GENEO_DLS1_SINGLE_STEP_ROWS")) : 4000000;
    const int tail = (int64_t)nL >= single_rows ? 1 : 2;
    while (!done && it < opt.dls1_max_it) run(tail);
    if (it == first && first > 8) cg_long_len = first - 2;
    else if (it >= first + 4) cg_long_len = first + 2;
  } else {
    while (!done && it < opt.dls1_max_it) run(check);
    if (use_amg && adaptive && done && cg_long_len == 0 && check % 2 == 0) {
      const int len = ((it - check - 2) / 2) * 2;
      cg_long_len = len >= 8 ? len : -1;
    }
  }
  info.dls1_iterations += it;
  info.dls1_solves += 1;
  if (dbg_dls1) {
    fprintf(stderr, "[dls1] solve %lld: %d iterations (first chunk %d), subdomains frozen at", info.dls1_solves, it, cg_long_len);
    for (int s = 0; s < ns; ++s) fprintf(stderr, " %d", conv_at[s]);
    fprintf(stderr, "\n");
  }
  if (!done) throw std::runtime_error("GenEO - solve KO: dls1 (KSP_DIVERGED_ITS)");
  if (opt.lvl1SRAS) bk::xmy(wL, x, d_D, nL);
  else bk::copy(wL, x, nL);
}

void PC::cheb_release() {
  cheb_chain.reset();
  bk::dfree(d_cheb_coef);
  d_cheb_coef = nullptr;
  cheb_work.release();
  cheb_K = 0;
  cheb_res_fused = 0;
  cheb_lo.clear();
  cheb_hi.clear();
  cheb_achieved.clear();
  cheb_its.clear();
}

std::vector<double> PC::cheb_table() const {
  std::vector<double> t((size_t)cheb_K * subs.size() * 2);
  if (!t.empty() && d_cheb_coef) bk::d2h(t.data(), d_cheb_coef, sizeof(double) * t.size());
  return t;
}

static void cheb_coefficients(double lo, double hi, int its, int K, int ns, int s, std::vector<double>& coef) {
  const double theta = 0.5 * (hi + lo), delta = 0.5 * (hi - lo);
  double rho = delta / theta;
  for (int k = 0; k < K; ++k) {
    double a = 0.0, b = 0.0;
    if (k == 0) {
      a = 1.0 / theta;
    } else if (k < its) {
      const double rho1 = 1.0 / (2.0 * theta / delta - rho);
      a = 2.0 * rho1 / delta;
      b = rho1 * rho;
      rho = rho1;
    }
    coef[((size_t)k * ns + s) * 2] = a;
    coef[((size_t)k * ns + s) * 2 + 1] = b;
  }
}

int PC::setup_cheb() {
  cheb_release();
  const int ns = (int)subs.size();
  if (!amg1) return fail("GenEO preconditioner: -dls1_ksp_type chebyshev needs the level-1 hierarchy (-dls1_pc_type amg)");
  if (ns == 0 || nL == 0) return 0;
  const int nlz = opt.dls1_cheb_esteig_its;
  if (!(opt.dls1_cheb_safety_lo > 0.0) || !(opt.dls1_cheb_safety_hi > 0.0))
    return fail("GenEO preconditioner: -dls1_cheb_safety needs two positive factors");
  struct Tmp {
    double *blk = nullptr, *rhs = nullptr, *nrm = nullptr;
    ~Tmp() { bk::dfree(blk); bk::dfree(rhs); bk::dfree(nrm); }
  } tmp;
  tmp.blk = (double*)bk::alloc(sizeof(double) * 2 * (size_t)nL);
  tmp.rhs = (double*)bk::alloc(sizeof(double) * (size_t)nL);
  tmp.nrm = (double*)bk::alloc(sizeof(double) * 2 * (size_t)ns);
  bk::block_init(ch, tmp.blk, 2, 2, d_subgid, 0x63686562ull);
  bk::block_axpby(tmp.rhs, 1, 1.0, tmp.blk + 1, 2, 0.0, nL, 1);
  std::vector<double> sc((size_t)8 * ns);
  std::vector<std::vector<double>> al(ns), be(ns);
  bk::cg_start(ch, d_cg_sc, d_xL, d_cg_r, d_cg_z, d_cg_p, tmp.rhs, nullptr);
  amg1->vcycle(d_cg_r, 1, d_cg_z, 1, 1);
  bk::seg_partial(ch, d_cg_r, d_cg_z, 1);
  bk::cg_set_rz(ch, d_cg_sc);
  bk::copy(d_cg_p, d_cg_z, nL);
  int parity = 0;
  for (int k = 0; k < nlz; ++k) {
    bk::spmv(dirL, d_cg_p, d_cg_q);
    bk::seg_pap(ch, d_cg_p, d_cg_q);
    bk::cg_update(ch, d_cg_sc, parity, d_xL, d_cg_r, d_cg_z, d_cg_p, d_cg_q, nullptr);
    amg1->vcycle(d_cg_r, 1, d_cg_z, 1, 1);
    bk::seg_partial(ch, d_cg_r, d_cg_z, 1);
    bk::cg_direction(ch, d_cg_sc, parity, d_cg_p, d_cg_z, 0.0);
    parity ^= 1;
    bk::d2h(sc.data(), d_cg_sc, sizeof(double) * 8 * ns);
    for (int s = 0; s < ns; ++s) {
      al[s].push_back(sc[(size_t)s * 8 + 4]);
      be[s].push_back(sc[(size_t)s * 8 + 5]);
    }
  }
  cheb_lo.assign(ns, 0.0);
  cheb_hi.assign(ns, 0.0);
  cheb_its.assign(ns, 0);
  int K = 0;
  for (int s = 0; s < ns; ++s) {
    int m = 0;
    while (m < nlz && std::isfinite(al[s][m]) && al[s][m] > 0.0) {
      ++m;
      if (!(std::isfinite(be[s][m - 1]) && be[s][m - 1] >= 0.0)) break;
    }
    if (m < 2)
      return fail("GenEO preconditioner: -dls1_ksp_type chebyshev: the bound estimate of subdomain " + std::to_string(subs[s].gid) +
                  " broke down after " + std::to_string(m) + " Lanczos step(s) (two are needed)");
    std::vector<double> T((size_t)m * m, 0.0), w, v;
    for (int k = 0; k < m; ++k) {
      T[(size_t)k * m + k] = 1.0 / al[s][k] + (k > 0 ? be[s][k - 1] / al[s][k - 1] : 0.0);
      if (k + 1 < m) T[(size_t)k * m + k + 1] = T[(size_t)(k + 1) * m + k] = std::sqrt(be[s][k]) / al[s][k];
    }
    dense::sym_eig(T, m, w, v);
    const double tmin = *std::min_element(w.begin(), w.end()), tmax = *std::max_element(w.begin(), w.end());
    const double lo = opt.dls1_cheb_safety_lo * tmin, hi = opt.dls1_cheb_safety_hi * tmax;
    if (!std::isfinite(lo) || !std::isfinite(hi) || !(lo > 0.0) || !(hi > lo))
      return fail("GenEO preconditioner: -dls1_ksp_type chebyshev: no usable bounds for subdomain " + std::to_string(subs[s].gid) +
                  " (Ritz values " + std::to_string(tmin) + " .. " + std::to_string(tmax) + ", -dls1_cheb_safety " +
                  std::to_string(opt.dls1_cheb_safety_lo) + "," + std::to_string(opt.dls1_cheb_safety_hi) + ")");
    const double sigma = (hi + lo) / (hi - lo);
    const int kcap = std::max(1, opt.dls1_max_it);
    int k = 1;
    double t0 = 1.0, t1 = sigma;
    while (k < kcap && !(1.0 / t1 <= opt.dls1_rtol)) {
      const double t2 = 2.0 * sigma * t1 - t0;
      t0 = t1;
      t1 = t2;
      ++k;
    }
    cheb_lo[s] = lo;
    cheb_hi[s] = hi;
    cheb_its[s] = k;
    K = std::max(K, k);
  }
  std::vector<double> coef((size_t)K * ns * 2, 0.0);
  for (int s = 0; s < ns; ++s) cheb_coefficients(cheb_lo[s], cheb_hi[s], cheb_its[s], K, ns, s, coef);
  d_cheb_coef = (double*)bk::alloc(sizeof(double) * coef.size());
  bk::h2d(d_cheb_coef, coef.data(), sizeof(double) * coef.size());
  cheb_K = K;
  cheb_work.alloc(nL, ns, 1);
  bk::copy(d_wL, tmp.rhs, nL);
  cheb_steps(vec, nullptr);
  bk::spmv(dirL, d_wL, d_cg_q);
  bk::axpy(d_cg_q, -1.0, tmp.rhs, nL);
  bk::seg_dot(ch, d_cg_q, d_cg_q, tmp.nrm, 2, 0);
  bk::seg_dot(ch, tmp.rhs, tmp.rhs, tmp.nrm, 2, 1);
  std::vector<double> nr((size_t)2 * ns);
  bk::d2h(nr.data(), tmp.nrm, sizeof(double) * 2 * ns);
  cheb_achieved.assign(ns, 0.0);
  for (int s = 0; s < ns; ++s) {
// ... 148 lines not shown
    prolong(a.wl, Y, w, a.ye);
    info.lvl2ApplyTimeLoc += secs(t0, t1);
    info.lvl1ApplyMinvTimeLoc += secs(t1, t2);
    info.lvl1ApplyTimeLoc += secs(t1, clk::now());
    return;
  }
  bool have_q = false;
  if (opt.lvl2 && !opt.effHybrid) {
    apply_q_on(a, X, Y);
    have_q = true;
    info.lvl2ApplyTimeLoc += secs(t0, clk::now());
  }
  auto t1 = clk::now();
  double* W = a.t1;
  bk::copy(W, X, nw);
  if (opt.hybrid && !opt.effHybrid) {
    matmult(Y, a.t2, w, a.wl, a.xe, a.ye);
    bk::axpy(W, -1.0, a.t2, nw);
  }
  restrict(W, a.wl, w, a.xe);
  auto t2 = clk::now();
  local_solve(a);
  info.lvl1ApplyMinvTimeLoc += secs(t2, clk::now());
  prolong(a.wl, W, w, a.ye);
  if (opt.hybrid) {
    matmult(W, a.t2, w, a.wl, a.xe, a.ye);
    apply_q_on(a, a.t2, a.t3);
    bk::axpy(W, -1.0, a.t3, nw);
  }
  if (have_q) bk::axpy(Y, 1.0, W, nw);
  else bk::copy(Y, W, nw);
  info.lvl1ApplyTimeLoc += secs(t1, clk::now());
}

int PC::apply_q(const double* x, double* y) {
  if (!is_setup || !opt.lvl2) return fail("GenEO preconditioner: no coarse space");
  try {
    apply_q_on(vec, x, y);
  } catch (std::exception& e) {
    return fail(e.what());
  }
  return 0;
}

int PC::apply(const double* x, double* y) {
  if (!is_setup) return fail("GenEO preconditioner is not set up");
  try {
    apply_on(vec, x, y);
  } catch (std::exception& e) {
    return fail(e.what());
  }
  return 0;
}

void PC::block_release() {
  blk_chain.reset();
  slab = App{};
  void* ptrs[] = {blk_r0, blk_r1, blk_z, blk_d, blk_x, blk_in, blk_out, blk_t1, blk_t2, blk_t3, blk_xe, blk_yE, blk_G,
                  blk_C, blk_ZR, blk_col, blk_dots, blk_dotwork, blk_coef, blk_g2e, blk_e2c};
  for (void* p : ptrs) bk::dfree(p);
  blk_r0 = blk_r1 = blk_z = blk_d = blk_x = blk_in = blk_out = blk_t1 = blk_t2 = blk_t3 = blk_xe = nullptr;
  blk_yE = blk_G = blk_C = blk_ZR = blk_col = blk_dots = blk_dotwork = blk_coef = nullptr;
  blk_g2e = blk_e2c = nullptr;
  blk_work.release();
  for (double* p : blk_basis) bk::dfree(p);
  blk_basis.clear();
  for (void* p : {(void*)blk_basis_tab, (void*)blk_gs_h, (void*)blk_gs_c, (void*)blk_gs_work}) bk::dfree(p);
  blk_basis_tab = nullptr;
  blk_gs_h = blk_gs_c = blk_gs_work = nullptr;
  blk_gs_bytes = 0.0;
  blk_gs_fused = blk_gs_composed = 0;
  blk_w = blk_kp = 0;
  blk_slabs = blk_columns = blk_padded = 0;
  coarse_blk_blocked = coarse_blk_by_column = coarse_blk_host = 0;
}

int PC::setup_block() {
  block_release();
  const int w = opt.block_width;
  if (w == 0) return 0;
  if (opt.dls1_ksp != "chebyshev" || !amg1) return fail("GenEO preconditioner: -geneo_block_width needs -dls1_ksp_type chebyshev");
  const int ns = (int)subs.size(), nown = n_owned();
  slab_entries(std::max(nL, std::max(nE, nown)), w);
  auto dv = [](size_t n) { return (double*)bk::alloc(sizeof(double) * std::max<size_t>(1, n)); };
  for (double** p : {&blk_r0, &blk_r1, &blk_z, &blk_d, &blk_x}) *p = dv((size_t)nL * w);
  for (double** p : {&blk_in, &blk_out, &blk_t1, &blk_t2, &blk_t3}) *p = dv((size_t)nown * w);
  blk_xe = dv((size_t)std::max(nE, nown) * w);
  blk_dots = dv(w);
  blk_coef = dv(2 * (size_t)w);
  blk_dotwork = dv((size_t)bk::BLOCK_COLDOT_WG * w);
  if (opt.lvl2 && dimE > 0 && d_Z) {
    const int kp = ((std::max(1, kmax) + 15) / 16) * 16;
    blk_kp = kp;
    blk_ZR = dv((size_t)nL * kp);
    bk::z_rowmajor(ch, d_Z, d_zbase, d_ksub, blk_ZR, kp);
    blk_yE = dv(((size_t)dimE + 1) * w);
    blk_G = dv(((size_t)ns * kp + 1) * w);
    blk_C = dv((size_t)std::max(1, ns) * kp * w);
    blk_col = dv(dimE);
    bk::zero(blk_yE + (size_t)dimE * w, sizeof(double) * w);
    bk::zero(blk_G + (size_t)ns * kp * w, sizeof(double) * w);
    std::vector<int> g2e(dimE, ns * kp), e2c((size_t)std::max(1, ns) * kp, dimE);
    for (int s = 0; s < ns; ++s)
      for (int k = 0; k < ksub[s]; ++k) {
        g2e[zoff[s] + k] = s * kp + k;
        e2c[(size_t)s * kp + k] = zoff[s] + k;
      }
    blk_g2e = (int*)bk::alloc(sizeof(int) * g2e.size());
    blk_e2c = (int*)bk::alloc(sizeof(int) * e2c.size());
    bk::h2d(blk_g2e, g2e.data(), sizeof(int) * g2e.size());
    bk::h2d(blk_e2c, e2c.data(), sizeof(int) * e2c.size());
  }
  blk_w = w;
  slab.w = w;
  slab.coarse = blk_ZR != nullptr;
  slab.wl = blk_r0; slab.xl = blk_x; slab.r1 = blk_r1; slab.z = blk_z; slab.d = blk_d;
  slab.t1 = blk_t1; slab.t2 = blk_t2; slab.t3 = blk_t3;
  slab.xe = slab.ye = blk_xe;
  slab.work = &blk_work;
  slab.chain = &blk_chain;
  return 0;
}

void PC::block_info(int* width, long long* slabs, long long* columns, long long* padded, long long* graph_launches) const {
  if (width) *width = blk_w;
  if (slabs) *slabs = blk_slabs;
  if (columns) *columns = blk_columns;
  if (padded) *padded = blk_padded;
  if (graph_launches) *graph_launches = blk_chain.replays;
}

void PC::block_krylov_info(int* basis_slabs, double* basis_bytes, long long* gs_fused, long long* gs_composed) const {
  if (basis_slabs) *basis_slabs = (int)blk_basis.size();
  if (basis_bytes) *basis_bytes = blk_gs_bytes;
  if (gs_fused) *gs_fused = blk_gs_fused;
  if (gs_composed) *gs_composed = blk_gs_composed;
}

void PC::coarse_block_counters(long long* blocked, long long* by_column, long long* host_blocks) const {
  if (blocked) *blocked = coarse_blk_blocked;
  if (by_column) *by_column = coarse_blk_by_column;
  if (host_blocks) *host_blocks = coarse_blk_host;
}

int PC::block_check(const char* who, int ld, int m, const void* a, const void* b) {
  if (!is_setup) return fail(std::string(who) + ": GenEO preconditioner is not set up");
  if (blk_w == 0) return fail(std::string(who) + ": the preconditioner was set up without -geneo_block_width (16 or 32)");
  if (m < 1) return fail(std::string(who) + ": the block needs at least one column");
  if (ld < n_owned()) return fail(std::string(who) + ": leading dimension " + std::to_string(ld) + " is below the " +
                                  std::to_string(n_owned()) + " owned rows");
  if (!a || !b) return fail(std::string(who) + ": null block");
  return 0;
}

void PC::slab_in(const double* Xcm, int ld, int m, double* slab) {
  if (g_block_fused.load()) bk::block_import(Xcm, ld, n_owned(), m, slab, blk_w);
  else block_import_composed(Xcm, ld, n_owned(), m, slab, blk_w);
}
void PC::slab_out(const double* slab, int m, double* Ycm, int ld) {
  if (g_block_fused.load()) bk::block_export(slab, blk_w, n_owned(), m, Ycm, ld);
  else block_export_composed(slab, blk_w, n_owned(), m, Ycm, ld);
}

int PC::slab_loop(bool apply, const double* X, int ldx, double* Y, int ldy, int m) {
  if (int rc = block_check(apply ? "PCMatApply_GenEO" : "MatMatMult_GenEO", std::min(ldx, ldy), m, X, Y)) return rc;
  try {
// ... 220 lines not shown
      end = s1;
      pending = s1 - s0;
      perr = &err;
      ++generation;
    }
    cv.notify_all();
    work();
    std::unique_lock<std::mutex> lk(mu);
    done_cv.wait(lk, [&] { return pending == 0; });
    fn = nullptr;
    if (err) std::rethrow_exception(err);
  }
  ~HostPool() {
    {
      std::unique_lock<std::mutex> lk(mu);
      stop = true;
    }
    cv.notify_all();
    for (auto& t : workers) t.join();
  }

 private:
  HostPool() {
    const unsigned hw = std::max(1u, std::thread::hardware_concurrency());
    const int n = (int)std::min(15u, hw > 1 ? hw - 1 : 0u);
    for (int i = 0; i < n; ++i)
      workers.emplace_back([this]() {
        unsigned long long seen = 0;
        for (;;) {
          {
            std::unique_lock<std::mutex> lk(mu);
            cv.wait(lk, [&] { return stop || generation != seen; });
            if (stop) return;
            seen = generation;
          }
          work();
        }
      });
  }
  void work() {
    for (;;) {
      int s;
      const std::function<void(int)>* f;
      {
        std::unique_lock<std::mutex> lk(mu);
        if (!fn || next >= end) return;
        s = next++;
        f = fn;
      }
      in_pool_work = true;
      try {
        (*f)(s);
      } catch (...) {
        std::unique_lock<std::mutex> lk(mu);
        if (perr && !*perr) *perr = std::current_exception();
      }
      in_pool_work = false;
      std::unique_lock<std::mutex> lk(mu);
      if (--pending == 0) done_cv.notify_all();
    }
  }
  std::vector<std::thread> workers;
  std::mutex run_mu;
  static thread_local bool in_pool_work;
  std::mutex mu;
  std::condition_variable cv, done_cv;
  const std::function<void(int)>* fn = nullptr;
  std::exception_ptr* perr = nullptr;
  int next = 0, end = 0, pending = 0;
  unsigned long long generation = 0;
  bool stop = false;
};

thread_local bool HostPool::in_pool_work = false;

int PC::lobpcg_solve(const EigProblem& P, int m, std::vector<double>& lam, double* Xc) {
  const int ns = (int)subs.size();
  const int nL = P.rows >= 0 ? P.rows : this->nL;
  const bk::Chunks& ch = P.chunks ? *P.chunks : this->ch;
  auto rows_of = [&](int s) { return P.row_off ? P.row_off[s + 1] - P.row_off[s] : (int)subs[s].l2g.size(); };
  const int nev_try = P.nev_try;
  const int p3 = 3 * m;
  const size_t blk = (size_t)nL * p3;
  auto dv = [](size_t n) { return (double*)bk::alloc(sizeof(double) * std::max<size_t>(1, n)); };
  double *S = dv(blk), *AS = dv(blk), *BS = dv(blk), *T = dv(blk), *AT = dv(blk), *BT = dv(blk);
  double *cr = dv((size_t)nL * m), *cd = dv((size_t)nL * m), *cad = dv((size_t)nL * m);
  double *dGA = dv((size_t)ns * p3 * p3), *dGB = dv((size_t)ns * p3 * p3), *dC = dv((size_t)ns * p3 * 2 * m);
  double* dGW = dv((size_t)ns * 2 * m * p3);
  double *dlam = dv((size_t)ns * m), *dnr = dv((size_t)ns * m), *dna = dv((size_t)ns * m), *dnb = dv((size_t)ns * m);
  std::vector<double*> owned_bufs = {S, AS, BS, T, AT, BT, cr, cd, cad, dGA, dGB, dGW, dC, dlam, dnr, dna, dnb};
  void** graphs_to_free = nullptr;
  bk::Chunks* groups_to_free = nullptr;
  void** events_to_free = nullptr;
  auto cleanup = [&]() {
    for (double* p : owned_bufs) bk::dfree(p);
    for (int i = 0; i < 2; ++i) {
      if (groups_to_free && groups_to_free[i].start) bk::chunks_free(groups_to_free[i]);
      if (events_to_free && events_to_free[i]) bk::event_destroy(events_to_free[i]);
    }
    if (graphs_to_free)
      for (int i = 0; i < 2; ++i) bk::graph_destroy(graphs_to_free[i]);
  };

  auto applyA = [&](const double* X, double* Y) { bk::spmm_strided(*P.A, X, p3, Y, p3, m, P.As, P.As); info.eig_spmm++; };
  auto applyB = [&](const double* X, double* Y) { bk::spmm_strided(*P.B, X, p3, Y, p3, m, P.Bs, P.Bs); info.eig_spmm++; };

  std::vector<double> hGA((size_t)ns * p3 * p3), hGB((size_t)ns * p3 * p3);
  struct Pinned {
    double* p = nullptr;
    size_t n = 0;
    explicit Pinned(size_t count) : p((double*)bk::pinned_alloc(sizeof(double) * std::max<size_t>(1, count))), n(count) {
      std::fill(p, p + n, 0.0);
    }
    ~Pinned() { bk::pinned_free(p); }
    Pinned(const Pinned&) = delete;
    Pinned& operator=(const Pinned&) = delete;
    double* data() { return p; }
    double* begin() { return p; }
  };
  Pinned hC((size_t)ns * p3 * 2 * m), hKL((size_t)ns * 2 * m);
  Pinned hGw((size_t)ns * 2 * m * p3);
  bool have_prop = false;
  bool fused_update = false;
  bool have_R = false;
  bool lean = false;
  std::vector<double> keep((size_t)ns * m, 1.0);
  double* dkeep = nullptr;
  static const bool full_gram = getenv("GENEO_LOBPCG_FULL_GRAM") != nullptr;
  std::vector<double> nr((size_t)ns * m), na((size_t)ns * m), nb((size_t)ns * m);
  std::vector<std::vector<double>> res(ns, std::vector<double>(m, 1.0));
  lam.assign((size_t)ns * m, 0.0);

  double* dGd = nullptr;
  if (P.defl && !P.defl->empty()) {
    int kmax_d = 0;
    for (auto& b : *P.defl) kmax_d = std::max(kmax_d, b.k);
    dGd = dv((size_t)ns * kmax_d * m);
    owned_bufs.push_back(dGd);
  }
  auto deflate = [&](double* Q, int ld) {
    if (!dGd) return;
    for (auto& b : *P.defl) {
      bk::gram(ch, b.BY, b.k, b.k, Q, ld, m, dGd);
      bk::axpby(dGd, -1.0, dGd, 0.0, ns * b.k * m);
      bk::block_mul(ch, b.Y, b.k, b.k, dGd, m, Q, ld, true);
    }
  };
  if (P.X0) bk::block_axpby(S, p3, 1.0, P.X0, m, 0.0, nL, m);
  else bk::block_init(ch, S, p3, m, d_subgid, opt.eps_seed + (uint64_t)P.seed_off);
  deflate(S, p3);
  applyA(S, AS);
  applyB(S, BS);
  std::vector<char> frozen(ns, 0), locked((size_t)ns * m, 0);
  if (P.skip)
    for (int s = 0; s < ns; ++s) frozen[s] = P.skip[s] ? 1 : 0;
  std::vector<double> mask((size_t)ns * m, 1.0);
  double* dmask = dv((size_t)ns * m);
  owned_bufs.push_back(dmask);
  bk::h2d(dmask, mask.data(), sizeof(double) * mask.size());
  dkeep = dv((size_t)ns * m);
  owned_bufs.push_back(dkeep);
  void* it_graph[2] = {nullptr, nullptr};
  bool graph_has_gram[2] = {true, true};
  static const bool want_pipeline = getenv("GENEO_LOBPCG_PIPELINE") != nullptr;
  const bool pipeline_ok = ns >= 2 && want_pipeline;
  int grp[3] = {0, ns, ns};
  bk::Chunks chg[2];
  void* gram_ev[2] = {nullptr, nullptr};
  if (pipeline_ok) {
// ... 61 lines not shown
            const double cka = ck[a];
            if (cka == 0.0) continue;
            double* oa = out + (size_t)a * p3;
            for (int b = 0; b < qout; ++b) oa[b] += cka * tk[b];
          }
        }
      }
    });
    t_prop_host += secs(tg, clk::now());
  };
  auto rayleigh_ritz = [&](int p, int nfix, int qout, bool with_p, int s0 = 0, int s1 = -1, const bk::Chunks* cg = nullptr,
                           bool last = true) -> int {
    if (s1 < 0) s1 = ns;
    if (!cg) cg = &ch;
    auto tg1 = clk::now();
    std::fill(hC.begin() + (size_t)s0 * p * qout, hC.begin() + (size_t)s1 * p * qout, 0.0);
    const bool want_prop = (p == p3) && conv_sinvert_now;
    auto rr_one = [&](int s) {
      std::vector<double> ga(hGA.begin() + (size_t)s * p * p, hGA.begin() + (size_t)(s + 1) * p * p);
      std::vector<double> gb(hGB.begin() + (size_t)s * p * p, hGB.begin() + (size_t)(s + 1) * p * p);
      for (int a = 0; a < p; ++a)
        for (int b = a + 1; b < p; ++b) {
          ga[a * p + b] = ga[b * p + a] = 0.5 * (ga[a * p + b] + ga[b * p + a]);
          gb[a * p + b] = gb[b * p + a] = 0.5 * (gb[a * p + b] + gb[b * p + a]);
        }
      if (want_prop) {
        std::copy(ga.begin(), ga.end(), hSA.begin() + (size_t)s * p * p);
        std::copy(gb.begin(), gb.end(), hSB.begin() + (size_t)s * p * p);
      }
      double* cs = hC.data() + (size_t)s * p * qout;
      if (frozen[s]) {
        for (int j = 0; j < m; ++j) cs[(size_t)j * qout + j] = 1.0;
        return;
      }
      std::vector<double> th, C;
      const int r = dense::gen_eig_rr(ga, gb, p, nfix, opt.rr_drop, th, C);
      for (int j = 0; j < m; ++j) {
        if (j < r) {
          lam[(size_t)s * m + j] = th[j];
          for (int i = 0; i < p; ++i) {
            const double v = C[(size_t)i * r + j];
            cs[(size_t)i * qout + j] = v;
            if (with_p && i >= m && !locked[(size_t)s * m + j]) cs[(size_t)i * qout + m + j] = v;
          }
        } else {
          lam[(size_t)s * m + j] = 1e300;
        }
      }
    };
    on_host_threads(rr_one, s0, s1);
    if (want_prop && last) {
      prop_pending = true;
      have_prop = true;
    }
    t_rr_host += secs(tg1, clk::now());
    const size_t co = (size_t)s0 * p * qout, mo = (size_t)s0 * m;
    bk::h2d_async(dC + co, hC.data() + co, sizeof(double) * (size_t)(s1 - s0) * p * qout);
    if (fused_update && p == p3 && with_p) {
      for (size_t e = mo; e < (size_t)s1 * m; ++e) keep[e] = (locked[e] || frozen[e / m]) ? 0.0 : 1.0;
      double* hk = hKL.data() + mo;
      double* hl = hKL.data() + (size_t)ns * m + mo;
      std::copy(keep.begin() + mo, keep.begin() + (size_t)s1 * m, hk);
      std::copy(lam.begin() + mo, lam.begin() + (size_t)s1 * m, hl);
      bk::h2d_async(dkeep + mo, hk, sizeof(double) * (size_t)(s1 - s0) * m);
      bk::h2d_async(dlam + mo, hl, sizeof(double) * (size_t)(s1 - s0) * m);
      if (lean) bk::lobpcg_update32_basis(*cg, S, dC + co, dkeep + mo, T);
      else bk::lobpcg_update32(*cg, S, AS, BS, dC + co, dkeep + mo, dlam + mo, dmask + mo, T, AT, BT, cr);
      if (last) have_R = true;
    } else {
      if (s0 != 0 || s1 != ns) throw std::runtime_error("lobpcg: grouped update without the fused kernel");
      have_R = false;
      bk::block_mul(ch, S, p3, p, dC, qout, T, p3, false);
      bk::block_mul(ch, AS, p3, p, dC, qout, AT, p3, false);
      bk::block_mul(ch, BS, p3, p, dC, qout, BT, p3, false);
    }
    if (last) {
      std::swap(S, T);
      if (!lean) { std::swap(AS, AT); std::swap(BS, BT); }
    }
    return 0;
  };
  gram_blocks(m);
  rayleigh_ritz(m, 0, m, false);
  bk::block_axpby(S + m, p3, 0.0, S + m, p3, 0.0, nL, m);
  bk::block_axpby(AS + m, p3, 0.0, AS + m, p3, 0.0, nL, m);
  bk::block_axpby(BS + m, p3, 0.0, BS + m, p3, 0.0, nL, m);

  const double tol = P.tol > 0.0 ? P.tol : opt.eps_tol;
  const double lmax = P.lmax * 1.05, lmin = lmax / std::max(1.5, opt.cheb_ratio);
  const double theta = 0.5 * (lmax + lmin), delta = 0.5 * (lmax - lmin), sigma = theta / delta;
  const bool conv_sinvert = P.amg && opt.eps_conv != "residual";
  conv_sinvert_now = conv_sinvert;
  fused_update = conv_sinvert && m == 32 && bk::lobpcg_update32_available() && !getenv("GENEO_LOBPCG_NO_FUSED_UPDATE");
  static const bool no_lean = getenv("GENEO_LOBPCG_NO_LEAN") != nullptr;
  lean = fused_update && !no_lean && !pipeline_ok && !full_gram && P.dual_pat && bk::spmm_dual_available(*P.dual_pat, m);
  if (getenv("GENEO_DEBUG") && !lean)
    fprintf(stderr, "[lobpcg %s] carried form: shift-invert test %d, block %d, fused update %d, shared pattern %d\n", P.label,
            (int)conv_sinvert, m, (int)fused_update, (int)(P.dual_pat != nullptr));
  if (lean) {
    for (double* q : {AT, BT}) {
      owned_bufs.erase(std::find(owned_bufs.begin(), owned_bufs.end(), q));
      bk::dfree(q);
    }
    AT = BT = nullptr;
  }
  int it = 0;
  bool all_done = false;
  std::vector<int> nev_s(ns);
  for (int s = 0; s < ns; ++s)
    nev_s[s] = std::max(0, std::min(nev_try, rows_of(s) - (P.locked_cols ? P.locked_cols[s] : 0)));
  static const bool nolock = getenv("GENEO_LOBPCG_NOLOCK") != nullptr;
  std::vector<double> lam_prev((size_t)ns * m, 1e300);
  static const bool lock_at_tol = getenv("GENEO_LOBPCG_LOCK_AT_TOL") != nullptr;
  const double tol_lock = lock_at_tol ? tol : std::max(tol * tol, std::min(tol, 1e-10));
  std::vector<char> conv((size_t)ns * m, 0);
  auto update_locks = [&](int s0 = 0, int s1 = -1) {
    bool done = true;
    if (s1 < 0) s1 = ns;
    for (int s = s0; s < s1; ++s) {
      if (frozen[s]) continue;
      bool sub_done = true;
      for (int j = 0; j < m; ++j) {
        const size_t e = (size_t)s * m + j;
        if (lam[e] >= 1e299 || (res[s][j] <= tol_lock && !nolock)) locked[e] = 1;
        if (lam[e] >= 1e299 || res[s][j] <= tol) conv[e] = 1;
        if (j < nev_s[s] && !conv[e]) sub_done = false;
      }
      if (sub_done && conv_sinvert && !nolock && nev_s[s] >= 1 && nev_s[s] < m) {
        static const double slack = getenv("GENEO_LOBPCG_SLACK") ? atof(getenv("GENEO_LOBPCG_SLACK")) : 2.0;
        const double last = lam[(size_t)s * m + nev_s[s] - 1] * (1.0 - slack * tol);
        for (int j = nev_s[s]; j < m; ++j) {
          const size_t e = (size_t)s * m + j;
          if (conv[e] || lam[e] >= 1e299) continue;
          const double drop = (lam_prev[e] < 1e299) ? std::max(0.0, lam_prev[e] - lam[e]) : lam[e];
          if (lam[e] / (1.0 + res[s][j]) > last) continue;
          if (lam[e] - 12.0 * drop > last) continue;
          sub_done = false;
        }
      }
      if (sub_done) frozen[s] = 1;
      else done = false;
    }
    return done;
  };
  auto debug_line = [&]() {
    if (!getenv("GENEO_DEBUG")) return;
    fprintf(stderr, "[lobpcg %s] it %d maxres:", P.label, it);
    for (int s = 0; s < ns; ++s) {
      double mx = 0.0;
      for (int j = 0; j < nev_s[s]; ++j) mx = std::max(mx, res[s][j]);
      fprintf(stderr, " %.2e", mx);
    }
    fprintf(stderr, " | locked");
    for (int s = 0; s < ns; ++s) {
      int nl = 0;
      for (int j = 0; j < m; ++j) nl += locked[(size_t)s * m + j] ? 1 : 0;
      fprintf(stderr, " %d", nl);
    }
    fprintf(stderr, " | prefix");
    for (int s = 0; s < ns; ++s) {
      int k = 0;
      while (k < m && (locked[(size_t)s * m + k] || frozen[s])) ++k;
      fprintf(stderr, " %d", k);
    }
    fprintf(stderr, " | lam0 %.6e %.6e .. %.6e | pc %s\n", lam[0], lam[1], lam[std::max(1, nev_s[0]) - 1], P.amg ? "amg" : "cheb");
  };
  const int max_it = P.max_it > 0 ? P.max_it : opt.eps_max_it;
  for (it = 0; it <= max_it; ++it) {
    static const int refresh = getenv("GENEO_LOBPCG_REFRESH") ? atoi(getenv("GENEO_LOBPCG_REFRESH")) : 8;
// ... 175 lines not shown
  if (opt.noSyl && cut > 0) nev = std::min(opt.eps_nev, cut);
  if (opt.noSyl && cut <= 0) nev = opt.eps_nev;
  if (nev_try) *nev_try = nev;
  if (opt.eps_block > 0) return opt.eps_block;
  const int want = nev + std::max(4, nev / 4);
  return want <= 16 ? 16 : (want <= 32 ? 32 : 64);
}

int PC::eig_block_max() const {
  if (opt.cut <= 0 && !opt.noSyl && opt.eps_block <= 0) return 64;
  return eig_targets(nullptr);
}

void PC::local_tau() {
  const int ns = (int)subs.size();
  tauLoc.assign(ns, opt.tau);
  if (opt.cst) return;
  for (int s = 0; s < ns; ++s) {
    int k = 0;
    for (int v : subs[s].mult) k = std::max(k, v);
    double t = k * opt.tau;
    if (t >= 1.0) t = 0.9;
    tauLoc[s] = t;
  }
}

int PC::local_gamma() {
  const int ns = (int)subs.size(), Pn = nsub_global;
  gammaLoc.assign(ns, opt.gamma);
  if (opt.cst) return 0;
  std::vector<double> c((size_t)Pn * Pn, 0.0);
  bool have_all = true;
  for (auto& s : subs) have_all = have_all && (int)s.intersect.size() == Pn;
  if (!have_all) {
    if (size > 1) return fail("GenEO-2: intersection flags are required on several ranks (PCGenEOSetIntersect), or use -geneo_cst");
    std::vector<std::vector<int>> owners(N);
    for (int s = 0; s < ns; ++s)
      for (int g : subs[s].l2g) owners[g].push_back(s);
    for (auto& s : subs) s.intersect.assign(Pn, 0);
    for (auto& o : owners)
      for (int a : o)
        for (int b : o)
          if (a != b) subs[a].intersect[subs[b].gid] = 1;
  }
  for (auto& s : subs)
    for (int q = 0; q < Pn; ++q) c[(size_t)s.gid * Pn + q] = (q == s.gid) ? 1.0 : (s.intersect[q] ? 0.0 : 1.0);
  if (size > 1) {
    double* dc = (double*)bk::alloc(sizeof(double) * c.size());
    bk::h2d(dc, c.data(), sizeof(double) * c.size());
    allreduce(dc, (int)c.size());
    bk::d2h(c.data(), dc, sizeof(double) * c.size());
    bk::dfree(dc);
  }
  std::vector<double> f(Pn), mth((size_t)Pn * Pn);
  for (int r = 0; r < Pn; ++r) {
    double sum = 0.0;
    for (int q = 0; q < Pn; ++q) sum += c[(size_t)r * Pn + q];
    f[r] = 1.0 / sum;
  }
  for (int r = 0; r < Pn; ++r)
    for (int q = 0; q < Pn; ++q)
      mth[(size_t)r * Pn + q] = 0.5 * (c[(size_t)r * Pn + q] + c[(size_t)q * Pn + r]) * f[r] * f[q];
  std::vector<double> w, V;
  dense::sym_eig(mth, Pn, w, V);
  double lmax = w[0];
  for (double v : w)
    if (std::fabs(v) > std::fabs(lmax)) lmax = v;
  for (int s = 0; s < ns; ++s) {
    double g = opt.gamma / lmax;
    g = g * f[subs[s].gid] * f[subs[s].gid];
    if (g <= 1.0) g = 1.1;
    gammaLoc[s] = g;
  }
  return 0;
}

int PC::eigen_lobpcg() {
  const int ns = (int)subs.size();
  const bool g2 = (opt.lvl2 == 2);
  int nev_try = 0;
  const int m = eig_targets(&nev_try);
  if (m != 16 && m != 32 && m != 64) return fail("GenEO: -els2_eps_block must be 16, 32 or 64");
  if (nev_try > m) return fail("GenEO: -geneo_cut / -els2_eps_nev larger than the LOBPCG block (max 64)");
  auto dv = [](size_t n) { return (double*)bk::alloc(sizeof(double) * std::max<size_t>(1, n)); };
  bk::Csr dirB = dirL;
  bool own_dirB = false;
  if (opt.lvl1ORAS) {
    std::vector<const HostCsr*> dm(ns);
    for (int s = 0; s < ns; ++s) dm[s] = &subs[s].a_dir;
    dirB = upload_blockdiag(dm, suboff, nullptr);
    dirB.fine = true;
    own_dirB = true;
  }
  bk::Csr dirBD = bk::csr_scaled_alias(dirB, d_D, d_D, false);
  double* neu_on_dir = (!g2 && !getenv("GENEO_LOBPCG_NO_DUAL")) ? bk::sell_values_on(dirB, neuL) : nullptr;
  auto release = [&]() {
    if (neu_on_dir) bk::dfree(neu_on_dir);
    neu_on_dir = nullptr;
    bk::csr_free(dirBD);
    if (own_dirB) bk::csr_free(dirB);
  };
  info.eig_iterations = 0;
  std::vector<HostCsr> robh;
  std::vector<const HostCsr*> hostB(ns);
  if (opt.check) {
    if (g2) robh.resize(ns);
    for (int s = 0; s < ns; ++s) {
      if (g2) {
        make_robin(subs[s], robh[s]);
        hostB[s] = &robh[s];
      } else {
        hostB[s] = &subs[s].a_dir;
      }
    }
  }
  struct Stage {
    double* X = nullptr;
    int m = 0;
    std::vector<double> lam;
    std::vector<int> count;
  };
  std::vector<double*> lock_bufs;
  auto free_stages = [&](std::vector<Stage>& st) {
    for (auto& g : st)
      if (g.X) bk::dfree(g.X);
    st.clear();
  };
  auto solve_grow = [&](EigProblem P, bool gamma, std::vector<Stage>& out) -> int {
    int mm = m, nev = nev_try;
    auto wanted = [&](int s, double l) { return gamma ? (l > 0.0 && 1.0 / l >= gammaLoc[s]) : (l <= tauLoc[s]); };
    Stage cur;
    for (;;) {
      P.nev_try = nev;
      cur.X = dv((size_t)nL * mm);
      cur.m = mm;
      if (int rc = lobpcg_solve(P, mm, cur.lam, cur.X)) { bk::dfree(cur.X); return rc; }
      P.X0 = nullptr;
      cur.count.assign(ns, 0);
      for (int s = 0; s < ns; ++s) cur.count[s] = std::min(nev, (int)subs[s].l2g.size());
      if (opt.cut > 0 || opt.noSyl || opt.eps_block > 0) { out.push_back(cur); return 0; }
      bool full = false;
      for (int s = 0; s < ns; ++s) {
        const int n_s = (int)subs[s].l2g.size(), nv = cur.count[s];
        if (nv >= n_s) continue;
        const double last = cur.lam[(size_t)s * mm + nv - 1];
        if (last < 1e299 && wanted(s, last)) full = true;
      }
      if (!full) { out.push_back(cur); return 0; }
      if (nev >= 48) break;
      bk::dfree(cur.X);
      cur.X = nullptr;
      nev = std::min(48, 2 * nev);
      const int want = nev + std::max(4, nev / 4);
      mm = want <= 16 ? 16 : (want <= 32 ? 32 : 64);
    }
    const double tight = std::min(opt.eps_tol, 1e-8);
    if (tight < opt.eps_tol) {
      P.tol = tight;
      P.nev_try = nev;
      if (int rc = lobpcg_solve(P, mm, cur.lam, cur.X)) { bk::dfree(cur.X); return rc; }
    }
    std::vector<EigProblem::Locked> locked_blocks;
    std::vector<int> locked_cols(ns, 0);
    std::vector<char> skip(ns, 0);
    for (int stage = 1;; ++stage) {
      std::vector<double> cs((size_t)ns * cur.m, 0.0);
      bool any = false;
      for (int s = 0; s < ns; ++s) {
        const int n_s = (int)subs[s].l2g.size(), nv = cur.count[s];
        bool full = !skip[s] && nv > 0 && locked_cols[s] + nv < n_s;
        if (full) {
          const double last = cur.lam[(size_t)s * cur.m + nv - 1];
          full = last < 1e299 && wanted(s, last);
        }
        if (!full) { skip[s] = 1; continue; }
        any = true;
        for (int j = 0; j < nv; ++j) cs[(size_t)s * cur.m + j] = 1.0;
        locked_cols[s] += nv;
        if (locked_cols[s] + 48 > 256) {
          out.push_back(cur);
          return fail("GenEO: more than 256 eigenvalues pass the threshold in one subdomain (coarse-space kernels hold 256 "
                      "vectors per subdomain): set -geneo_cut or lower -geneo_tau");
        }
      }
      out.push_back(cur);
      if (!any) return 0;
      double* Y = dv((size_t)nL * cur.m);
      double* BY = dv((size_t)nL * cur.m);
      lock_bufs.push_back(Y);
      lock_bufs.push_back(BY);
      {
        struct DevBuf { double* p; ~DevBuf() { bk::dfree(p); } } dcs{dv(cs.size())};
        bk::h2d(dcs.p, cs.data(), sizeof(double) * cs.size());
        bk::block_axpby(Y, cur.m, 1.0, cur.X, cur.m, 0.0, nL, cur.m);
        bk::block_colscale(ch, Y, cur.m, cur.m, dcs.p);
        bk::spmm_strided(*P.B, Y, cur.m, BY, cur.m, cur.m, P.Bs, P.Bs);
        bk::sync();
      }
      locked_blocks.push_back({Y, BY, cur.m});
      Stage nxt;
      nxt.m = 64;
      nxt.X = dv((size_t)nL * 64);
      EigProblem Pd = P;
      Pd.nev_try = 48;
      Pd.defl = &locked_blocks;
      Pd.skip = skip.data();
      Pd.locked_cols = locked_cols.data();
      Pd.seed_off = stage;
      if (int rc = lobpcg_solve(Pd, 64, nxt.lam, nxt.X)) { bk::dfree(nxt.X); return rc; }
      nxt.count.assign(ns, 0);
      for (int s = 0; s < ns; ++s)
        if (!skip[s]) nxt.count[s] = std::max(0, std::min(48, (int)subs[s].l2g.size() - locked_cols[s]));
      cur = nxt;
    }
  };
  info.eig_coarse_iterations = 0;
  struct DevBlock {
    double* p = nullptr;
    ~DevBlock() { if (p) bk::dfree(p); }
    double* release() { double* q = p; p = nullptr; return q; }
  };
  struct CsrHold {
    bk::Csr c;
    bool live = false;
    void drop() { if (live) bk::csr_free(c); live = false; }
    ~CsrHold() { drop(); }
  };
  struct ChunksHold {
    bk::Chunks c;
    ~ChunksHold() { if (c.start) bk::chunks_free(c); }
  };
  std::function<double*(int, const bk::Csr&)> start_block = [&](int l, const bk::Csr& Bl) -> double* {
    if (l + 1 >= amgN->nlevels()) return nullptr;
    const int min_rows = getenv("GENEO_COARSE_START_MIN_ROWS") ? atoi(getenv("GENEO_COARSE_START_MIN_ROWS")) : 4096;
    const double ctol = getenv("GENEO_COARSE_START_TOL") ? atof(getenv("GENEO_COARSE_START_TOL")) : 1e-2;
    const std::vector<int>& co = amgN->level_suboff(l + 1);
    const int nc = amgN->level_rows(l + 1);
    bool fits = (int)co.size() == ns + 1;
    for (int s = 0; fits && s < ns; ++s) fits = co[s + 1] - co[s] >= std::max(4 * m, l == 0 ? 0 : min_rows);
    if (!fits) return nullptr;
    const auto t0 = clk::now();
    CsrHold BP, Bc;
    bool ok = true;
    BP.c = bk::spgemm(Bl, amgN->level_P(l), nc, &ok);
    BP.live = ok;
    if (!ok) return nullptr;
    Bc.c = bk::spgemm(amgN->level_R(l), BP.c, nc, &ok);
    Bc.live = ok;
    BP.drop();
    if (!ok) return nullptr;
    bk::csr_finish(Bc.c);
    DevBlock below, Xc, X0;
    below.p = start_block(l + 1, Bc.c);
    const auto t1 = clk::now();
    ChunksHold cc;
    cc.c = bk::chunks_upload(ns, co.data());
    EigProblem pc{&amgN->level_A(l + 1), nullptr, &Bc.c, nullptr, amgN, amgN->level_dinv(l + 1), cheb_lmax, nev_try, "tau-coarse"};
    pc.rows = nc;
    pc.chunks = &cc.c;
    pc.row_off = co.data();
    pc.amg_level = l + 1;
    pc.tol = std::max(opt.eps_tol, ctol);
    pc.iterations = &info.eig_coarse_iterations;
    pc.max_it = 40;
    pc.X0 = below.p;
    std::vector<double> lamc;
    Xc.p = dv((size_t)nc * m);
    const int before = info.eig_coarse_iterations;
    const int rc = lobpcg_solve(pc, m, lamc, Xc.p);
    if (rc) last_error.clear();
    bool full = rc == 0;
    for (size_t e = 0; full && e < lamc.size(); ++e) full = lamc[e] < 1e299;
    if (full) {
      X0.p = dv((size_t)amgN->level_rows(l) * m);
      bk::spmm_strided(amgN->level_P(l), Xc.p, m, X0.p, m, m, nullptr, nullptr);
    }
    if (getenv("GENEO_DEBUG")) {
      bk::sync();
      fprintf(stderr, "[coarse start] level %d: %d rows, B products + levels below %.3f s, %d LOBPCG iterations + prolongation %.3f s%s\n",
              l + 1, nc, secs(t0, t1), info.eig_coarse_iterations - before, secs(t1, clk::now()), full ? "" : " -- not used");
    }
    return X0.release();
  };
  auto coarse_start = [&]() -> double* {
    if (g2 || !amgN || opt.els2_pc != "amg" || opt.eig_coarse_start <= 0 || ns == 0) return nullptr;
    if (!(opt.cut > 0 || opt.noSyl || opt.eps_block > 0)) return nullptr;
    if (amgN->level_rows(0) != nL) return nullptr;
    for (int s = 0; s < ns; ++s)
      if ((int64_t)subs[s].l2g.size() < (int64_t)opt.eig_coarse_start) return nullptr;
    return start_block(0, dirBD);
  };
  std::vector<Stage> stT, stG;
  auto release_all = [&]() {
    free_stages(stT);
    free_stages(stG);
    for (double* q : lock_bufs) bk::dfree(q);
    lock_bufs.clear();
    release();
  };
  {
    EigProblem pt{&neuL, nullptr, g2 ? &dirL : &dirBD, nullptr, (opt.els2_pc == "amg") ? amgN : nullptr,
                  d_dinvN, cheb_lmax, nev_try, "tau"};
    if (neu_on_dir && dirBD.sl_val) {
      pt.dual_pat = &dirB;
      pt.dual_vA = neu_on_dir;
      pt.dual_vB = dirBD.sl_val;
    }
    if (opt.check)
      if (int rc = check_local_spd(pt, hostB.data(), !g2)) { release_all(); return rc; }
    double* X0 = coarse_start();
    pt.X0 = X0;
    const int rc_tau = solve_grow(pt, false, stT);
    if (X0) bk::dfree(X0);
    if (rc_tau) { release_all(); return rc_tau; }
  }
  if (g2) {
    if (int rc = local_gamma()) { release_all(); return rc; }
    if (int rc = finish_amg1()) { release_all(); return rc; }
    EigProblem pg{&dirL, nullptr, &dirBD, nullptr, (opt.els2_pc == "amg" && opt.dls1_pc == "amg") ? amg1 : nullptr,
                  d_dinv1, cheb_lmax1, nev_try, "gamma"};
    if (opt.check) {
      EigProblem pchk = pg;
      pchk.B = &dirL;
      pchk.Bs = nullptr;
      if (int rc = check_local_spd(pchk, hostB.data(), false)) { release_all(); return rc; }
    }
    if (int rc = solve_grow(pg, true, stG)) { release_all(); return rc; }
  }
  for (double* q : lock_bufs) bk::dfree(q);
  lock_bufs.clear();
  auto make_sel = [&](const std::vector<Stage>& st) {
    std::vector<std::vector<int>> v(st.size());
    for (size_t g = 0; g < st.size(); ++g) v[g].assign((size_t)ns * (st[g].m + 1), 0);
    return v;
  };
  std::vector<std::vector<int>> selT = make_sel(stT), selG = make_sel(stG);
  std::vector<std::vector<int>> kT(stT.size(), std::vector<int>(ns, 0)), kG(stG.size(), std::vector<int>(ns, 0));
  std::vector<std::vector<double>> gscale(stG.size());
  for (size_t g = 0; g < stG.size(); ++g) gscale[g].assign((size_t)ns * stG[g].m, 1.0);
  ksub.assign(ns, 0);
  double* ones = d_cg_p;
  double* tmp = d_cg_q;
  bk::set(ones, 1.0, nL);
  bk::spmv(neuL, ones, tmp);
  bk::seg_dot(ch, tmp, ones, d_cg_sc, 8, 0);
  if (g2) {
    bk::spmv(dirL, ones, tmp);
  } else {
    bk::xmy(d_cg_r, ones, d_D, nL);
    bk::spmv(dirB, d_cg_r, tmp);
    bk::xmy(tmp, tmp, d_D, nL);
  }
  bk::seg_dot(ch, tmp, ones, d_cg_sc, 8, 1);
  std::vector<double> sc((size_t)8 * ns);
  bk::d2h(sc.data(), d_cg_sc, sizeof(double) * 8 * ns);
  for (int s = 0; s < ns; ++s) {
    int cnt = 0;
// ... 437 lines not shown
  for (int j = 0; j < dimE; ++j) {
    unit[j] = 1.0;
    bk::h2d(d_yE, unit.data(), sizeof(double) * dimE);
    unit[j] = 0.0;
    bk::z_apply(ch, d_Z, d_zbase, d_ksub, d_zoff, d_yE, d_wL, false);
    prolong(d_wL, d_t1, 1, d_ye);
    restrict(d_t1, d_xL, 1, d_xe);
    bk::zt_apply(ch, d_Z, d_zbase, d_ksub, d_zoff, kmax, d_xL, d_yE, dimE);
    allreduce(d_yE, dimE);
    bk::d2h(colv.data(), d_yE, sizeof(double) * dimE);
    for (int i = 0; i < dimE; ++i) G[(size_t)i * dimE + j] = colv[i];
  }
  std::vector<double> R((size_t)dimE * dimE, 0.0);
  int bad = -1;
  for (int i = 0; i < dimE && bad < 0; ++i) {
    double d = G[(size_t)i * dimE + i];
    for (int t = 0; t < i; ++t) d -= R[(size_t)t * dimE + i] * R[(size_t)t * dimE + i];
    if (!(d > DBL_EPSILON * DBL_EPSILON * G[(size_t)i * dimE + i])) { bad = i; break; }
    const double rii = std::sqrt(d);
    R[(size_t)i * dimE + i] = rii;
    for (int j = i + 1; j < dimE; ++j) {
      double v = 0.5 * (G[(size_t)i * dimE + j] + G[(size_t)j * dimE + i]);
      for (int t = 0; t < i; ++t) v -= R[(size_t)t * dimE + i] * R[(size_t)t * dimE + j];
      R[(size_t)i * dimE + j] = v / rii;
    }
  }
  if (rank == 0) {
    std::ofstream f("check.setup.ZE2G.R");
    f.precision(16);
    for (int i = 0; i < dimE; ++i) {
      for (int j = 0; j < dimE; ++j) f << (j ? " " : "") << R[(size_t)i * dimE + j];
      f << std::endl;
    }
  }
  if (bad >= 0) {
    std::ostringstream msg;
    msg << "GenEO - check rank: Z = Q*R with R(" << bad << ", " << bad << ") = 0";
    return fail(msg.str());
  }
  return 0;
}

int PC::build_E() {
  const int ns = (int)subs.size();
  std::vector<double> kg(std::max(1, nsub_global), 0.0);
  for (int s = 0; s < ns; ++s) {
    if (subs[s].gid < 0 || subs[s].gid >= nsub_global) return fail("GenEO: bad global subdomain id");
    kg[subs[s].gid] = ksub[s];
  }
  if (size > 1) {
    double* dk = (double*)bk::alloc(sizeof(double) * nsub_global);
    bk::h2d(dk, kg.data(), sizeof(double) * nsub_global);
    allreduce(dk, nsub_global);
    bk::d2h(kg.data(), dk, sizeof(double) * nsub_global);
    bk::dfree(dk);
  }
  ksub_global.assign(nsub_global, 0);
  std::vector<int> zoff_g(nsub_global + 1, 0);
  for (int g = 0; g < nsub_global; ++g) {
    ksub_global[g] = (int)std::lround(kg[g]);
    zoff_g[g + 1] = zoff_g[g] + ksub_global[g];
  }
  dimE = zoff_g[nsub_global];
  info.dimE = dimE;
  info.realDimELoc = 0;
  kmax = 0;
  zoff.assign(ns, 0);
  for (int s = 0; s < ns; ++s) {
    zoff[s] = zoff_g[subs[s].gid];
    kmax = std::max(kmax, ksub[s]);
    info.realDimELoc += ksub[s];
  }
  d_ksub = (int*)bk::alloc(sizeof(int) * std::max(1, ns));
  d_zoff = (int*)bk::alloc(sizeof(int) * std::max(1, ns));
  bk::h2d(d_ksub, ksub.data(), sizeof(int) * ns);
  bk::h2d(d_zoff, zoff.data(), sizeof(int) * ns);
  d_yE = (double*)bk::alloc(sizeof(double) * std::max(1, dimE));
  h_yE.assign(std::max(1, dimE), 0.0);
  E.assign((size_t)dimE * dimE, 0.0);
  const int nown = n_owned();
  const int W = std::min(32, size == 1 ? 32 : comm_width);
  if (W >= 8 && dimE > 0 && !getenv("GENEO_E_COLUMNWISE")) {
    const int kp = ((std::max(1, kmax) + 15) / 16) * 16;
    auto dv = [](size_t n) { return (double*)bk::alloc(sizeof(double) * std::max<size_t>(1, n)); };
    double* ZR = dv((size_t)nL * kp);
    double *WLb = dv((size_t)nL * W), *XLb = dv((size_t)nL * W);
    double *T1 = dv((size_t)nown * W), *T2 = dv((size_t)nown * W);
    double* xe = dv((size_t)std::max(nE, nown) * W);
    double *dC = dv((size_t)ns * kp * W), *dG = dv((size_t)ns * kp * W);
    std::vector<double> hC((size_t)ns * kp * W), hG((size_t)ns * kp * W);
    bk::z_rowmajor(ch, d_Z, d_zbase, d_ksub, ZR, kp);
    int rc = 0;
    for (int j0 = 0; j0 < dimE && !rc; j0 += W) {
      std::fill(hC.begin(), hC.end(), 0.0);
      for (int s = 0; s < ns; ++s)
        for (int k = 0; k < ksub[s]; ++k) {
          const int c = zoff[s] + k - j0;
          if (c >= 0 && c < W) hC[((size_t)s * kp + k) * W + c] = 1.0;
        }
      bk::h2d(dC, hC.data(), sizeof(double) * hC.size());
      bk::block_mul(ch, ZR, kp, kp, dC, W, WLb, W, false);
      prolong(WLb, T1, W, xe);
      matmult(T1, T2, W, WLb, xe, xe);
      restrict(T2, XLb, W, xe);
      bk::gram(ch, ZR, kp, kp, XLb, W, W, dG);
      bk::d2h(hG.data(), dG, sizeof(double) * hG.size());
      for (int s = 0; s < ns; ++s)
        for (int k = 0; k < ksub[s]; ++k)
          for (int c = 0; c < W && j0 + c < dimE; ++c)
            E[(size_t)(zoff[s] + k) * dimE + j0 + c] = hG[((size_t)s * kp + k) * W + c];
    }
    for (double* p : {ZR, WLb, XLb, T1, T2, xe, dC, dG}) bk::dfree(p);
    if (size > 1) {
      double* dE = dv(E.size());
      bk::h2d(dE, E.data(), sizeof(double) * E.size());
      allreduce(dE, (int)E.size());
      bk::d2h(E.data(), dE, sizeof(double) * E.size());
      bk::dfree(dE);
    }
  } else {
  std::vector<double> unit(dimE, 0.0), colv(dimE);
  for (int j = 0; j < dimE; ++j) {
    unit[j] = 1.0;
    bk::h2d(d_yE, unit.data(), sizeof(double) * dimE);
    unit[j] = 0.0;
    bk::z_apply(ch, d_Z, d_zbase, d_ksub, d_zoff, d_yE, d_wL, false);
    prolong(d_wL, d_t1, 1, d_ye);
    matmult(d_t1, d_t2, 1, d_wL, d_xe, d_ye);
    restrict(d_t2, d_xL, 1, d_xe);
    bk::zt_apply(ch, d_Z, d_zbase, d_ksub, d_zoff, kmax, d_xL, d_yE, dimE);
    allreduce(d_yE, dimE);
    bk::d2h(colv.data(), d_yE, sizeof(double) * dimE);
    for (int i = 0; i < dimE; ++i) E[(size_t)i * dimE + j] = colv[i];
  }
  }
  (void)nown;
  Efac = E;
  for (int a = 0; a < dimE; ++a)
    for (int b = a + 1; b < dimE; ++b) Efac[(size_t)a * dimE + b] = Efac[(size_t)b * dimE + a] =
        0.5 * (Efac[(size_t)a * dimE + b] + Efac[(size_t)b * dimE + a]);
  const bool want_dev = dimE > 0 && (opt.coarse_device == Options::COARSE_ALWAYS ||
                                     (opt.coarse_device == Options::COARSE_AUTO && dimE > 1024));
  if (want_dev && factor_E_on_device(Efac)) {
    E_chol = true;
    Efac.clear();
    EfacT.clear();
    return 0;
  }
  std::vector<double> sym = Efac;
  E_chol = dense::cholesky_blocked(Efac, dimE, (int)std::min(16u, std::max(1u, std::thread::hardware_concurrency())));
  if (E_chol) {
    EfacT.assign(Efac.size(), 0.0);
    for (int a = 0; a < dimE; ++a)
      for (int b = 0; b <= a; ++b) EfacT[(size_t)b * dimE + a] = Efac[(size_t)a * dimE + b];
  }
  if (E_chol && dimE > 0 && dimE <= 1024 && !want_dev) {
    d_EL = (double*)bk::alloc(sizeof(double) * Efac.size());
    d_ELT = (double*)bk::alloc(sizeof(double) * EfacT.size());
    bk::h2d(d_EL, Efac.data(), sizeof(double) * Efac.size());
    bk::h2d(d_ELT, EfacT.data(), sizeof(double) * EfacT.size());
  }
  if (!E_chol) {
    Efac = sym;
    if (!dense::lu_factor(Efac, dimE, Epiv)) return fail("GenEO - solve KO: dcs2 (singular coarse operator E)");
  }
  return 0;
}

bool PC::factor_E_on_device(const std::vector<double>& sym) {
  double *dL = nullptr, *dLT = nullptr;
  int* dst = nullptr;
// ... 505 lines not shown
```

Baseline: 6408.

## Skip zero-fill for fully overwritten device buffers and add wave-level short-row sort

Adds an uninitialized f64 allocation path that skips the hipMemsetAsync zero-fill, and uses it for CSR values, AMG level buffers, LOBPCG blocks and E-construction work arrays that are fully written before being read. It also adds a single-wavefront register sort for transpose and SpGEMM rows of at most 64 entries, so the shared-memory bitonic sort only runs when longer rows exist. Allocation-site tracing and a poison option are added for debugging. The risk is reading garbage if any of these buffers was relying on the implicit zeroing. The LOBPCG axpby calls are changed so they read from a separate buffer instead of the now-uninitialized columns.

Result: no change. 6491 (median of 4 runs) (+1.3%).

```diff
diff --git a/geneo4petsc_amd/csrc/alloc_dev.h b/geneo4petsc_amd/csrc/alloc_dev.h
--- /dev/null
+++ b/geneo4petsc_amd/csrc/alloc_dev.h
@@ -0,0 +1,25 @@
+#pragma once
+
+#include <cstddef>
+
+#include "backend.h"
+
+namespace bk {
+
+double* alloc_f64_uninit(size_t n);
+
+const char* alloc_site(const char* tag);
+
+struct AllocSiteScope {
+  const char* prev;
+  explicit AllocSiteScope(const char* tag) : prev(alloc_site(tag)) {}
+  ~AllocSiteScope() { alloc_site(prev); }
+  AllocSiteScope(const AllocSiteScope&) = delete;
+  AllocSiteScope& operator=(const AllocSiteScope&) = delete;
+};
+
+}
+
+#define BK_SITE_CAT2(a, b) a##b
+#define BK_SITE_CAT(a, b) BK_SITE_CAT2(a, b)
+#define BK_ALLOC_SITE(tag) ::bk::AllocSiteScope BK_SITE_CAT(bk_alloc_site_, __LINE__)(tag)
diff --git a/geneo4petsc_amd/csrc/amg.cpp b/geneo4petsc_amd/csrc/amg.cpp
--- a/geneo4petsc_amd/csrc/amg.cpp
+++ b/geneo4petsc_amd/csrc/amg.cpp
@@ -13,6 +13,7 @@
 #include <stdexcept>
 #include <thread>
 
+#include "alloc_dev.h"
 #include "dense.h"
 
 namespace geneo {
@@ -613,13 +614,14 @@
 }
 
 void AmgDevice::alloc_level_buffers(Lvl& L, bool coarse) {
-  const size_t blk = sizeof(double) * std::max<size_t>(1, (size_t)L.n * maxm);
-  L.r = (double*)bk::alloc(blk);
-  L.d = (double*)bk::alloc(blk);
-  if (prm.smooth_degree > 1) L.ad = (double*)bk::alloc(blk);
+  const size_t blk = std::max<size_t>(1, (size_t)L.n * maxm);
+  BK_ALLOC_SITE("amg.level_buffers");
+  L.r = bk::alloc_f64_uninit(blk);
+  L.d = bk::alloc_f64_uninit(blk);
+  if (prm.smooth_degree > 1) L.ad = bk::alloc_f64_uninit(blk);
   if (coarse) {
-    L.b = (double*)bk::alloc(blk);
-    L.x = (double*)bk::alloc(blk);
+    L.b = bk::alloc_f64_uninit(blk);
+    L.x = bk::alloc_f64_uninit(blk);
   }
 }
 
diff --git a/geneo4petsc_amd/csrc/backend_hip.hip b/geneo4petsc_amd/csrc/backend_hip.hip
--- a/geneo4petsc_amd/csrc/backend_hip.hip
+++ b/geneo4petsc_amd/csrc/backend_hip.hip
@@ -17,6 +17,7 @@
 #include <unordered_map>
 #include <vector>
 
+#include "alloc_dev.h"
 #include "backend.h"
 #include "cheb_dev.h"
 
@@ -175,7 +176,29 @@
   g_cache_bytes = 0;
   g_free_s += std::chrono::duration<double>(std::chrono::high_resolution_clock::now() - t0).count();
 }
-void* alloc(size_t bytes) {
+static bool g_alloc_poison = false;
+static thread_local const char* t_alloc_site = nullptr;
+struct AllocSiteCount { long long calls = 0, filled = 0, unfilled = 0; };
+static std::map<std::string, AllocSiteCount> g_alloc_sites;
+static bool alloc_trace_on() {
+  static const bool on = getenv("GENEO_ALLOC_TRACE") != nullptr;
+  return on;
+}
+static void alloc_trace_dump() {
+  std::lock_guard<std::mutex> lk(g_alloc_mu);
+  std::vector<std::pair<std::string, AllocSiteCount>> v(g_alloc_sites.begin(), g_alloc_sites.end());
+  std::sort(v.begin(), v.end(), [](const auto& a, const auto& b) { return a.second.filled > b.second.filled; });
+  fprintf(stderr, "[alloc sites] %-28s %10s %14s %14s\n", "site", "calls", "filled MB", "unfilled MB");
+  for (const auto& kv : v)
+    fprintf(stderr, "[alloc sites] %-28s %10lld %14.1f %14.1f\n", kv.first.c_str(), kv.second.calls, kv.second.filled / 1e6,
+            kv.second.unfilled / 1e6);
+}
+const char* alloc_site(const char* tag) {
+  const char* prev = t_alloc_site;
+  t_alloc_site = tag;
+  return prev;
+}
+static void* alloc_block(size_t bytes, bool fill) {
   lazy_init();
   bind_thread();
   void* p = nullptr;
@@ -206,17 +229,27 @@
     }
     HIPCHK(e);
     const double dt = std::chrono::duration<double>(std::chrono::high_resolution_clock::now() - t0).count();
-    static const bool trace = getenv("GENEO_ALLOC_TRACE") != nullptr;
-    if (trace && dt > 2e-4) fprintf(stderr, "[alloc] %.1f MB in %.3f ms\n", sz / 1e6, dt * 1e3);
+    if (alloc_trace_on() && dt > 2e-4) fprintf(stderr, "[alloc] %.1f MB in %.3f ms\n", sz / 1e6, dt * 1e3);
     std::lock_guard<std::mutex> lk(g_alloc_mu);
     g_alloc_s += dt;
     ++g_alloc_n;
     g_live[p] = sz;
     mem_account((long long)sz);
   }
-  HIPCHK(hipMemsetAsync(p, 0, bytes, g_stream));
+  if (fill) HIPCHK(hipMemsetAsync(p, 0, bytes, g_stream));
+  else if (g_alloc_poison) HIPCHK(hipMemsetAsync(p, 0xFF, bytes, g_stream));
+  if (alloc_trace_on()) {
+    static const bool registered = (atexit(alloc_trace_dump), true);
+    (void)registered;
+    std::lock_guard<std::mutex> lk(g_alloc_mu);
+    AllocSiteCount& c = g_alloc_sites[t_alloc_site ? t_alloc_site : "(untagged)"];
+    ++c.calls;
+    (fill ? c.filled : c.unfilled) += (long long)bytes;
+  }
   return p;
 }
+void* alloc(size_t bytes) { return alloc_block(bytes, true); }
+double* alloc_f64_uninit(size_t n) { return (double*)alloc_block(sizeof(double) * n, false); }
 void dfree(void* p) {
   if (!p) return;
   bind_thread();
@@ -512,12 +545,13 @@
 static void finish_layout(Csr& a, const int* h_rowptr, const int* h_col = nullptr);
 
 Csr csr_upload_raw(int n, const int* h_rowptr, const int* h_col, const double* h_val) {
+  BK_ALLOC_SITE("csr_upload");
   Csr a;
   a.n = n;
   a.nnz = h_rowptr[n];
   a.rowptr = (int*)alloc(sizeof(int) * (size_t)(n + 1));
   a.col = (int*)alloc(sizeof(int) * std::max<size_t>(1, (size_t)a.nnz));
-  a.val = (double*)alloc(sizeof(double) * std::max<size_t>(1, (size_t)a.nnz));
+  a.val = alloc_f64_uninit(std::max<size_t>(1, (size_t)a.nnz));
   h2d(a.rowptr, h_rowptr, sizeof(int) * (size_t)(n + 1));
   h2d(a.col, h_col, sizeof(int) * (size_t)a.nnz);
   h2d(a.val, h_val, sizeof(double) * (size_t)a.nnz);
@@ -541,12 +575,13 @@
   return a;
 }
 Csr csr_upload(int n, const int* h_rowptr, const int* h_col, const double* h_val) {
+  BK_ALLOC_SITE("csr_upload");
   Csr a;
   a.n = n;
   a.nnz = h_rowptr[n];
   a.rowptr = (int*)alloc(sizeof(int) * (size_t)(n + 1));
   a.col = (int*)alloc(sizeof(int) * std::max<size_t>(1, (size_t)a.nnz));
-  a.val = (double*)alloc(sizeof(double) * std::max<size_t>(1, (size_t)a.nnz));
+  a.val = alloc_f64_uninit(std::max<size_t>(1, (size_t)a.nnz));
   static const bool dbg = getenv("GENEO_DEBUG") != nullptr;
   auto t0 = std::chrono::high_resolution_clock::now();
   h2d(a.rowptr, h_rowptr, sizeof(int) * (size_t)(n + 1));
@@ -681,6 +716,7 @@
 }
 
 static void finish_layout(Csr& a, const int* h_rowptr, const int* h_col) {
+  BK_ALLOC_SITE("csr_layout");
   const int n = a.n;
   static const bool dbg_l = getenv("GENEO_DEBUG") != nullptr;
   auto tl0 = std::chrono::high_resolution_clock::now();
@@ -1154,6 +1190,20 @@
   }
   __builtin_amdgcn_fence(__ATOMIC_ACQ_REL, "wavefront");
   __builtin_amdgcn_wave_barrier();
+  if (cnt <= 64) {
+    unsigned long long ck = ~0ull;
+    double v = 0.0;
+    if (lane < cnt) {
+      ck = (unsigned)list[w][lane];
+      v = lval[w][lane];
+    }
+    spg_sort64(ck, v, lane);
+    if (lane < cnt) {
+      ccol[base + lane] = (int)ck;
+      cval[base + lane] = v;
+    }
+    return;
+  }
   int N = 64;
   while (N < cnt) N <<= 1;
   wave_bitonic_sort(list[w], lval[w], N, lane);
@@ -1356,6 +1406,7 @@
 static bool g_spgemm_small_host = true;
 Csr spgemm(const Csr& a, const Csr& b, int ncols_b, bool* ok) {
   (void)ncols_b;
+  BK_ALLOC_SITE("spgemm");
   Csr c;
   *ok = true;
   t_sp_report = SparseProductReport();
@@ -1407,7 +1458,7 @@
   host_exclusive_scan(c.rowptr, a.n, &total);
   c.nnz = total;
   c.col = (int*)alloc(sizeof(int) * std::max<size_t>(1, (size_t)total));
-  c.val = (double*)alloc(sizeof(double) * std::max<size_t>(1, (size_t)total));
+  c.val = alloc_f64_uninit(std::max<size_t>(1, (size_t)total));
   if (G) SPG_SMALL_G(true);
   if (general) {
     if (g_spgemm_fill_scan)
@@ -1446,6 +1497,29 @@
       tval[p] = val[k];
     }
 }
+__global__ __launch_bounds__(256) void k_sort_rows_short(int n, const int* __restrict__ rp, int* __restrict__ col,
+                                                         double* __restrict__ val, int* __restrict__ flag) {
+  const int w = threadIdx.x >> 6, lane = threadIdx.x & 63;
+  const int row = blockIdx.x * 4 + w;
+  if (row >= n) return;
+  const int base = rp[row], cnt = rp[row + 1] - base;
+  if (cnt <= 1) return;
+  if (cnt > 64) {
+    if (lane == 0) flag[cnt > TR_MAXROW ? 0 : 1] = 1;
+    return;
+  }
+  unsigned long long ck = ~0ull;
+  double v = 0.0;
+  if (lane < cnt) {
+    ck = (unsigned)col[base + lane];
+    v = val[base + lane];
+  }
+  spg_sort64(ck, v, lane);
+  if (lane < cnt) {
+    col[base + lane] = (int)ck;
+    val[base + lane] = v;
+  }
+}
 __global__ __launch_bounds__(256) void k_sort_rows(int n, const int* __restrict__ rp, int* __restrict__ col,
                                                    double* __restrict__ val, int* __restrict__ overflow) {
   __shared__ int key[4][TR_MAXROW];
@@ -1454,7 +1528,7 @@
   const int row = blockIdx.x * 4 + w;
   if (row >= n) return;
   const int base = rp[row], cnt = rp[row + 1] - base;
-  if (cnt <= 1) return;
+  if (cnt <= 64) return;
   if (cnt > TR_MAXROW) {
     if (lane == 0) *overflow = 1;
     return;
@@ -1473,6 +1547,7 @@
   }
 }
 Csr transpose(const Csr& a, int ncols, bool* ok) {
+  BK_ALLOC_SITE("transpose");
   Csr t;
   *ok = true;
   t_sp_report = SparseProductReport();
@@ -1480,23 +1555,25 @@
   t.nnz = a.nnz;
   t.rowptr = (int*)alloc(sizeof(int) * ((size_t)ncols + 1));
   t.col = (int*)alloc(sizeof(int) * std::max<size_t>(1, (size_t)a.nnz));
-  t.val = (double*)alloc(sizeof(double) * std::max<size_t>(1, (size_t)a.nnz));
+  t.val = alloc_f64_uninit(std::max<size_t>(1, (size_t)a.nnz));
   if (a.nnz > 0)
     hipLaunchKernelGGL(k_col_count, dim3(gridv(a.nnz)), dim3(256), 0, g_stream, a.col, (int64_t)a.nnz, t.rowptr + 1);
   int64_t total = 0;
   host_exclusive_scan(t.rowptr, ncols, &total);
   int* cursor = (int*)alloc(sizeof(int) * std::max<size_t>(1, (size_t)ncols));
-  int* dflag = (int*)alloc(sizeof(int));
+  int* dflag = (int*)alloc(2 * sizeof(int));
   if (a.n > 0)
     hipLaunchKernelGGL(k_tr_scatter, dim3(gridv(a.n)), dim3(256), 0, g_stream, a.n, a.rowptr, a.col, a.val, t.rowptr,
                        cursor, t.col, t.val);
   if (ncols > 0)
+    hipLaunchKernelGGL(k_sort_rows_short, dim3((ncols + 3) / 4), dim3(256), 0, g_stream, ncols, t.rowptr, t.col, t.val, dflag);
+  int hflag[2] = {0, 0};
+  d2h(hflag, dflag, 2 * sizeof(int));
+  if (!hflag[0] && hflag[1])
     hipLaunchKernelGGL(k_sort_rows, dim3((ncols + 3) / 4), dim3(256), 0, g_stream, ncols, t.rowptr, t.col, t.val, dflag);
-  int hflag = 0;
-  d2h(&hflag, dflag, sizeof(int));
   dfree(dflag);
   dfree(cursor);
-  if (hflag) {
+  if (hflag[0]) {
     dfree(t.rowptr); dfree(t.col); dfree(t.val);
     *ok = false;
     return Csr();
@@ -1588,7 +1665,8 @@
   b.lp_val = nullptr; b.lp_col = nullptr; b.lp_base = nullptr;
   b.off_mask = nullptr; b.off_rec = nullptr; b.off_coded = 0; b.off_nnz = 0;
   b.col_scaled = col_is_dinv;
-  b.val = (double*)alloc(sizeof(double) * std::max<size_t>(1, (size_t)a.nnz));
+  BK_ALLOC_SITE("csr_scaled_alias");
+  b.val = alloc_f64_uninit(std::max<size_t>(1, (size_t)a.nnz));
   b.sl_val = (double*)alloc(sizeof(double) * (size_t)std::max<int64_t>(1, a.sl_nnz));
   if (a.n > 0)
     hipLaunchKernelGGL(k_scale_csr, dim3(grid1d(a.n, 256)), dim3(256), 0, g_stream, a.n, a.rowptr, a.col, a.val, row_scale,
@@ -2207,6 +2285,7 @@
   }
 }
 bool csr_make_lp(Csr& a, const Csr* index_owner) {
+  BK_ALLOC_SITE("csr_make_lp");
   if (spmv_kind() != 1 || a.nslice == 0 || !a.sl_ptr || a.vec_lpr > 0 || a.nlong > 0 || a.lp_val) return a.lp_val != nullptr;
   if (index_owner) {
     if (!index_owner->lp_val || index_owner->sl_col != a.sl_col) return false;
@@ -3003,6 +3082,7 @@
 }
 double* sell_values_on(const Csr& a, const Csr& b) {
   if (spmv_kind() != 1 || a.nlong > 0 || a.vec_lpr > 0 || !a.sl_ptr || a.n != b.n || a.nslice == 0) return nullptr;
+  BK_ALLOC_SITE("sell_values_on");
   double* out = (double*)alloc(sizeof(double) * (size_t)std::max<int64_t>(1, a.sl_nnz));
   int* dmiss = (int*)alloc(sizeof(int));
   hipLaunchKernelGGL(k_sell_values_on, dim3((a.nslice + 3) / 4), dim3(256), 0, g_stream, a.n, a.nslice, a.sl_ptr, a.sl_col,
@@ -4671,6 +4751,7 @@
     return true;
   }
   if (k == "sell_offsets") { g_sell_offsets = value != 0; return true; }
+  if (k == "alloc_poison") { g_alloc_poison = value != 0; return true; }
   if (k == "spgemm_small_rows") {
     lazy_init();
     const int off = value ? 0 : 1;
diff --git a/geneo4petsc_amd/csrc/core.cpp b/geneo4petsc_amd/csrc/core.cpp
--- a/geneo4petsc_amd/csrc/core.cpp
+++ b/geneo4petsc_amd/csrc/core.cpp
@@ -21,6 +21,7 @@
 #include <stdexcept>
 #include <thread>
 
+#include "alloc_dev.h"
 #include "amg.h"
 #include "block_dev.h"
 #include "cheb_dev.h"
@@ -33,6 +34,8 @@
 __attribute__((weak)) bool coarse_solve(const double*, const double*, int, int, double*) { return false; }
 __attribute__((weak)) bool coarse_solve_block(const double*, const double*, int, int, double*, int) { return false; }
 __attribute__((weak)) SparseProductReport sparse_product_report() { return SparseProductReport(); }
+__attribute__((weak)) double* alloc_f64_uninit(size_t n) { return (double*)alloc(sizeof(double) * n); }
+__attribute__((weak)) const char* alloc_site(const char*) { return nullptr; }
 }
 
 namespace geneo {
@@ -694,6 +697,7 @@
   for (int s = 0; s < ns; ++s) gids[s] = subs[s].gid;
   d_subgid = (int*)bk::alloc(sizeof(int) * std::max(1, ns));
   bk::h2d(d_subgid, gids.data(), sizeof(int) * ns);
+  BK_ALLOC_SITE("pc.work_vectors");
   auto dv = [](size_t n) { return (double*)bk::alloc(sizeof(double) * std::max<size_t>(1, n)); };
   d_xe = dv(nE); d_ye = dv(nE); d_xL = dv(nL); d_wL = dv(nL);
   d_cg_r = dv(nL); d_cg_z = dv(nL); d_cg_p = dv(nL); d_cg_q = dv(nL); d_cg_sc = dv((size_t)8 * std::max(1, ns));
@@ -1540,6 +1544,7 @@
     double *blk = nullptr, *rhs = nullptr, *nrm = nullptr;
     ~Tmp() { bk::dfree(blk); bk::dfree(rhs); bk::dfree(nrm); }
   } tmp;
+  BK_ALLOC_SITE("cheb_bounds.tmp");
   tmp.blk = (double*)bk::alloc(sizeof(double) * 2 * (size_t)nL);
   tmp.rhs = (double*)bk::alloc(sizeof(double) * (size_t)nL);
   tmp.nrm = (double*)bk::alloc(sizeof(double) * 2 * (size_t)ns);
@@ -1854,6 +1859,7 @@
   if (opt.dls1_ksp != "chebyshev" || !amg1) return fail("GenEO preconditioner: -geneo_block_width needs -dls1_ksp_type chebyshev");
   const int ns = (int)subs.size(), nown = n_owned();
   slab_entries(std::max(nL, std::max(nE, nown)), w);
+  BK_ALLOC_SITE("setup_block");
   auto dv = [](size_t n) { return (double*)bk::alloc(sizeof(double) * std::max<size_t>(1, n)); };
   for (double** p : {&blk_r0, &blk_r1, &blk_z, &blk_d, &blk_x}) *p = dv((size_t)nL * w);
   for (double** p : {&blk_in, &blk_out, &blk_t1, &blk_t2, &blk_t3}) *p = dv((size_t)nown * w);
@@ -2240,9 +2246,12 @@
   const int nev_try = P.nev_try;
   const int p3 = 3 * m;
   const size_t blk = (size_t)nL * p3;
+  BK_ALLOC_SITE("lobpcg_solve");
   auto dv = [](size_t n) { return (double*)bk::alloc(sizeof(double) * std::max<size_t>(1, n)); };
-  double *S = dv(blk), *AS = dv(blk), *BS = dv(blk), *T = dv(blk), *AT = dv(blk), *BT = dv(blk);
-  double *cr = dv((size_t)nL * m), *cd = dv((size_t)nL * m), *cad = dv((size_t)nL * m);
+  auto du = [](size_t n) { return bk::alloc_f64_uninit(std::max<size_t>(1, n)); };
+  double *S = du(blk), *AS = du(blk), *BS = du(blk), *T = du(blk), *AT = du(blk), *BT = du(blk);
+  double* cr = dv((size_t)nL * m);
+  double *cd = du((size_t)nL * m), *cad = du((size_t)nL * m);
   double *dGA = dv((size_t)ns * p3 * p3), *dGB = dv((size_t)ns * p3 * p3), *dC = dv((size_t)ns * p3 * 2 * m);
   double* dGW = dv((size_t)ns * 2 * m * p3);
   double *dlam = dv((size_t)ns * m), *dnr = dv((size_t)ns * m), *dna = dv((size_t)ns * m), *dnb = dv((size_t)ns * m);
@@ -2470,9 +2479,9 @@
   };
   gram_blocks(m);
   rayleigh_ritz(m, 0, m, false);
-  bk::block_axpby(S + m, p3, 0.0, S + m, p3, 0.0, nL, m);
-  bk::block_axpby(AS + m, p3, 0.0, AS + m, p3, 0.0, nL, m);
-  bk::block_axpby(BS + m, p3, 0.0, BS + m, p3, 0.0, nL, m);
+  bk::block_axpby(S + m, p3, 0.0, cr, m, 0.0, nL, m);
+  bk::block_axpby(AS + m, p3, 0.0, cr, m, 0.0, nL, m);
+  bk::block_axpby(BS + m, p3, 0.0, cr, m, 0.0, nL, m);
 
   const double tol = P.tol > 0.0 ? P.tol : opt.eps_tol;
   const double lmax = P.lmax * 1.05, lmin = lmax / std::max(1.5, opt.cheb_ratio);
@@ -2814,7 +2823,9 @@
   const int m = eig_targets(&nev_try);
   if (m != 16 && m != 32 && m != 64) return fail("GenEO: -els2_eps_block must be 16, 32 or 64");
   if (nev_try > m) return fail("GenEO: -geneo_cut / -els2_eps_nev larger than the LOBPCG block (max 64)");
+  BK_ALLOC_SITE("eigen_lobpcg");
   auto dv = [](size_t n) { return (double*)bk::alloc(sizeof(double) * std::max<size_t>(1, n)); };
+  auto du = [](size_t n) { return bk::alloc_f64_uninit(std::max<size_t>(1, n)); };
   bk::Csr dirB = dirL;
   bool own_dirB = false;
   if (opt.lvl1ORAS) {
@@ -2864,7 +2875,7 @@
     Stage cur;
     for (;;) {
       P.nev_try = nev;
-      cur.X = dv((size_t)nL * mm);
+      cur.X = du((size_t)nL * mm);
       cur.m = mm;
       if (int rc = lobpcg_solve(P, mm, cur.lam, cur.X)) { bk::dfree(cur.X); return rc; }
       P.X0 = nullptr;
@@ -2917,8 +2928,8 @@
       }
       out.push_back(cur);
       if (!any) return 0;
-      double* Y = dv((size_t)nL * cur.m);
-      double* BY = dv((size_t)nL * cur.m);
+      double* Y = du((size_t)nL * cur.m);
+      double* BY = du((size_t)nL * cur.m);
       lock_bufs.push_back(Y);
       lock_bufs.push_back(BY);
       {
@@ -2932,7 +2943,7 @@
       locked_blocks.push_back({Y, BY, cur.m});
       Stage nxt;
       nxt.m = 64;
-      nxt.X = dv((size_t)nL * 64);
+      nxt.X = du((size_t)nL * 64);
       EigProblem Pd = P;
       Pd.nev_try = 48;
       Pd.defl = &locked_blocks;
@@ -2997,14 +3008,14 @@
     pc.max_it = 40;
     pc.X0 = below.p;
     std::vector<double> lamc;
-    Xc.p = dv((size_t)nc * m);
+    Xc.p = du((size_t)nc * m);
     const int before = info.eig_coarse_iterations;
     const int rc = lobpcg_solve(pc, m, lamc, Xc.p);
     if (rc) last_error.clear();
     bool full = rc == 0;
     for (size_t e = 0; full && e < lamc.size(); ++e) full = lamc[e] < 1e299;
     if (full) {
-      X0.p = dv((size_t)amgN->level_rows(l) * m);
+      X0.p = du((size_t)amgN->level_rows(l) * m);
       bk::spmm_strided(amgN->level_P(l), Xc.p, m, X0.p, m, m, nullptr, nullptr);
     }
     if (getenv("GENEO_DEBUG")) {
@@ -3608,11 +3619,13 @@
   const int W = std::min(32, size == 1 ? 32 : comm_width);
   if (W >= 8 && dimE > 0 && !getenv("GENEO_E_COLUMNWISE")) {
     const int kp = ((std::max(1, kmax) + 15) / 16) * 16;
+    BK_ALLOC_SITE("build_E.work");
     auto dv = [](size_t n) { return (double*)bk::alloc(sizeof(double) * std::max<size_t>(1, n)); };
-    double* ZR = dv((size_t)nL * kp);
-    double *WLb = dv((size_t)nL * W), *XLb = dv((size_t)nL * W);
-    double *T1 = dv((size_t)nown * W), *T2 = dv((size_t)nown * W);
-    double* xe = dv((size_t)std::max(nE, nown) * W);
+    auto du = [](size_t n) { return bk::alloc_f64_uninit(std::max<size_t>(1, n)); };
+    double* ZR = du((size_t)nL * kp);
+    double *WLb = du((size_t)nL * W), *XLb = du((size_t)nL * W);
+    double *T1 = du((size_t)nown * W), *T2 = du((size_t)nown * W);
+    double* xe = du((size_t)std::max(nE, nown) * W);
     double *dC = dv((size_t)ns * kp * W), *dG = dv((size_t)ns * kp * W);
     std::vector<double> hC((size_t)ns * kp * W), hG((size_t)ns * kp * W);
     bk::z_rowmajor(ch, d_Z, d_zbase, d_ksub, ZR, kp);
```
